# tayloraswift/swift-png

Hardware: AMD Instinct MI355X
Metric: decoded_mpixels_per_s (higher is better)
Workload: dtype u8

## Files before the change

### include/spng_mi355.h

```cpp
#ifndef SPNG_MI355_H
#define SPNG_MI355_H

#include <stddef.h>
#include <stdint.h>

#ifdef __cplusplus
extern "C" {
#endif

#define SPNG_VERSION 0x000100

enum {
    SPNG_DONE = 0,
    SPNG_NEED_MORE_INPUT = 1,
    SPNG_E_COMPRESSION_METHOD = 16,
    SPNG_E_WINDOW_SIZE = 17,
    SPNG_E_CHECK_BITS = 18,
    SPNG_E_DICTIONARY = 19,
    SPNG_E_STREAM_CHECKSUM = 32,
    SPNG_E_BLOCK_TYPE = 33,
    SPNG_E_BLOCK_COUNT_PARITY = 34,
    SPNG_E_RUNLITERAL_COUNT = 35,
    SPNG_E_CODELENGTH_TABLE = 36,
    SPNG_E_CODELENGTH_SEQUENCE = 37,
// ... 3 lines not shown
    SPNG_E_GZIP_METHOD = 25,
    SPNG_E_GZIP_FLAG_BITS = 26,
    SPNG_E_GZIP_HEADER_CHECKSUM = 27,
    SPNG_E_EXTRANEOUS_IMAGE_DATA = 48,
    SPNG_E_EXTRANEOUS_COMPRESSED_DATA = 49,
    SPNG_E_INCOMPLETE_DATASTREAM = 50,
    SPNG_E_TRUNCATED_SIGNATURE = 80,
    SPNG_E_SIGNATURE = 81,
    SPNG_E_TRUNCATED_CHUNK_HEADER = 82,
    SPNG_E_TRUNCATED_CHUNK_BODY = 83,
    SPNG_E_CHUNK_TYPE = 84,
    SPNG_E_CHUNK_CHECKSUM = 85,
    SPNG_E_TEXT_KEYWORD = 96,
    SPNG_E_TEXT_CHUNK_LENGTH = 97,
    SPNG_E_TEXT_LANGUAGE = 98,
    SPNG_E_TEXT_LOCALIZED_KEYWORD = 99,
    SPNG_E_TEXT_COMPRESSION_METHOD = 100,
    SPNG_E_TEXT_COMPRESSION = 101,
    SPNG_E_TEXT_INCOMPLETE = 102,
    SPNG_E_PROFILE_NAME = 104,
    SPNG_E_PROFILE_CHUNK_LENGTH = 105,
    SPNG_E_PROFILE_COMPRESSION_METHOD = 106,
    SPNG_E_PROFILE_INCOMPLETE = 107,
    SPNG_E_TEXT_ENCODING = 112,
    SPNG_E_OUTPUT_CAPACITY = 64,
    SPNG_E_ARGUMENT = 65,
    SPNG_E_DEVICE = 66,
    SPNG_E_REFERENCE_UNDEFINED = 67
};

enum { SPNG_FORMAT_ZLIB = 0,
       SPNG_FORMAT_IOS = 1,
       SPNG_FORMAT_GZIP = 2 };

typedef struct spng_ctx spng_ctx;

typedef struct spng_result {
    int32_t  status;
    int32_t  reserved;
    uint64_t written;
    uint64_t consumed;
    uint64_t aux[2];
} spng_result;

typedef struct spng_stream_desc {
    const void *d_src;  uint64_t src_len;
    void       *d_dst;  uint64_t dst_cap;
    int32_t     format;
    int32_t     reserved;
} spng_stream_desc;

typedef struct spng_image_desc {
    const void *d_idat;    uint64_t idat_len;
    void       *d_rows;    uint64_t rows_cap;
    void       *d_storage;
    uint32_t    width, height;
    uint8_t     depth;
    uint8_t     channels;
    uint8_t     interlaced;
    uint8_t     format;
    uint32_t    reserved;
} spng_image_desc;
enum { SPNG_IMAGE_OVERDRAW = 1 };

int32_t     spng_version(void);
const char *spng_status_string(int32_t status);
const char *spng_last_error_string(void);
uint64_t    spng_inflated_size(uint32_t w, uint32_t h, int depth, int channels, int interlaced);
uint64_t    spng_storage_size(uint32_t w, uint32_t h, int depth, int channels);

int32_t spng_create(int device, void *stream, spng_ctx **out);
void    spng_destroy(spng_ctx *ctx);
void   *spng_stream(spng_ctx *ctx);
int32_t spng_sync(spng_ctx *ctx);

enum { SPNG_CFG_INFLATE_MODE = 0,
       SPNG_CFG_SEGMENT_BYTES = 1,
       SPNG_CFG_TOKEN_BYTES = 2,
       SPNG_CFG_UNFILTER_PIECE_ROWS = 3,
       SPNG_CFG_RESOLVE_PARTS = 5,
       SPNG_CFG_DEFLATE_BYTES = 7,
       SPNG_CFG_MULTI_GROUPS = 8,
       SPNG_CFG_BLOCK_CUT_BYTES = 9,
       SPNG_CFG_COUNT = 10 };
enum { SPNG_BLOCK_CUT_AUTO = 0, SPNG_BLOCK_CUT_NEVER = 1 };
enum { SPNG_INFLATE_AUTO = 0, SPNG_INFLATE_SERIAL = 1 };
int32_t spng_configure(spng_ctx *ctx, int key, int64_t value);

enum { SPNG_K_INFLATE = 0,
       SPNG_K_UNFILTER = 1, SPNG_K_SCATTER = 2, SPNG_K_FILTER = 3,
       SPNG_K_DEFLATE = 4, SPNG_K_ADLER = 5,
       SPNG_K_PINFLATE = 6,
       SPNG_K_UNPACK = 7,
       SPNG_K_PACK = 10,
       SPNG_K_LEX = 12,
       SPNG_K_PINF_FIND = 8, SPNG_K_PINF_DECODE = 9, SPNG_K_PINF_RESOLVE = 11,
       SPNG_K_DFL_SEARCH = 13, SPNG_K_DFL_PARSE = 14,
       SPNG_K_ALPHA = 15,
       SPNG_K_CENSUS = 16,
       SPNG_K_PACK_INDEXED = 17,
       SPNG_K_HSVA = 18,
       SPNG_K_LUMINANCE = 19,
       SPNG_K_COUNT = 19 + 1 };
int32_t spng_profile(spng_ctx *ctx, int enable);
int32_t spng_profile_get(spng_ctx *ctx, int kernel, double *total_ms, uint64_t *launches);
int32_t spng_token_stats(spng_ctx *ctx, uint64_t *page_bytes, uint64_t *blocks, int32_t *ran_dry);
int32_t spng_cut_stats(spng_ctx *ctx, uint64_t *tried, uint64_t *joined, uint64_t *streams_redone);

int32_t spng_inflate_batch(spng_ctx *ctx, const spng_stream_desc *descs, uint32_t count,
                           spng_result *d_results, spng_result *h_results);

int32_t spng_inflate_resume_batch(spng_ctx *ctx, const spng_stream_desc *descs, const uint64_t *h_state, uint32_t count,
                                  spng_result *d_results, spng_result *h_results);

int32_t spng_unfilter_batch(spng_ctx *ctx, const spng_image_desc *descs, uint32_t count,
                            const uint64_t *d_rows_len,
                            spng_result *d_results, spng_result *h_results);

int32_t spng_decode_batch(spng_ctx *ctx, const spng_image_desc *descs, uint32_t count,
                          spng_result *d_results, spng_result *h_results);

int32_t spng_inflate(spng_ctx *ctx, const void *src, uint64_t n, int32_t format,
                     void *dst, uint64_t cap, spng_result *result);
int32_t spng_unfilter(spng_ctx *ctx, const void *rows, uint64_t rows_len,
                      uint32_t w, uint32_t h, int depth, int channels, int interlaced,
                      void *storage, spng_result *result);
int32_t spng_decode(spng_ctx *ctx, const void *idat, uint64_t n, int32_t format,
                    uint32_t w, uint32_t h, int depth, int channels, int interlaced,
                    void *storage, spng_result *result);
int32_t spng_adler32(spng_ctx *ctx, const void *data, uint64_t n, uint32_t *out);

typedef struct spng_file_desc {
    const void *d_png;  uint64_t len;
    void       *d_idat; uint64_t idat_cap;
} spng_file_desc;
typedef struct spng_lexed {
    int32_t  status;
    uint32_t chunks;
    uint64_t aux[2];
    uint32_t width, height;
    uint8_t  depth, color, compression, filter, interlace;
    uint8_t  ios;
    uint8_t  pad[2];
    uint64_t idat_len;
    uint64_t plte_off, trns_off;
    uint32_t plte_len, trns_len;
    uint64_t consumed;
} spng_lexed;
int32_t spng_lex_batch(spng_ctx *ctx, const spng_file_desc *files, uint32_t count,
                       spng_lexed *d_infos, spng_lexed *h_infos);
uint64_t spng_lex_state_bytes(void);
int32_t spng_lex_resume_batch(spng_ctx *ctx, const spng_file_desc *files, void *const *d_states, uint32_t count,
                              spng_lexed *d_infos, spng_lexed *h_infos);
int32_t spng_lex_resume_stats(spng_ctx *ctx, uint64_t *summed, uint64_t *copied, uint64_t *headers);
#define SPNG_NO_OFFSET 0xffffffffu
typedef struct spng_chunk_entry {
    uint32_t type;
    uint32_t length;
    uint64_t offset;
    int32_t  status;
    uint32_t aux;
    uint32_t k, l, m;
    uint32_t body_off;
    uint8_t  compressed;
    uint8_t  pad[7];
} spng_chunk_entry;
typedef struct spng_chunk_dir {
    spng_chunk_entry *d_entries;
    uint32_t          cap;
    uint32_t          reserved;
} spng_chunk_dir;
int32_t spng_lex_dir_batch(spng_ctx *ctx, const spng_file_desc *files, const spng_chunk_dir *dirs, uint32_t count,
                           spng_lexed *d_infos, spng_lexed *h_infos);

enum { SPNG_TEXT_LATIN1_TO_UTF8 = 1,
       SPNG_TEXT_CHECK_UTF8 = 2 };
typedef struct spng_text_desc {
    const void *d_in;   uint64_t len;
    void       *d_out;  uint64_t out_cap;
    uint8_t     op;
    uint8_t     reserved[7];
} spng_text_desc;
int32_t spng_text_batch(spng_ctx *ctx, const spng_text_desc *descs, uint32_t count, spng_result *d_results, spng_result *h_results);

typedef struct spng_chunking_desc {
    const void *d_stream; uint64_t len;
    void       *d_out;    uint64_t out_cap;
    uint64_t    chunk_bytes;
} spng_chunking_desc;
int32_t spng_write_idat_batch(spng_ctx *ctx, const spng_chunking_desc *descs, uint32_t count,
// ... 205 lines not shown
```

### swift_png_amd/__init__.py

```python
from __future__ import annotations

import ctypes
import os
from pathlib import Path

_HERE = Path(__file__).resolve().parent
LIB_PATH = Path(os.environ.get("SPNG_LIB", _HERE / "libspng_mi355.so"))

DONE, NEED_MORE_INPUT = 0, 1
E_COMPRESSION_METHOD, E_WINDOW_SIZE, E_CHECK_BITS, E_DICTIONARY = 16, 17, 18, 19
E_GZIP_SIGIL, E_GZIP_METHOD, E_GZIP_FLAG_BITS, E_GZIP_HEADER_CHECKSUM = 24, 25, 26, 27
(E_STREAM_CHECKSUM, E_BLOCK_TYPE, E_BLOCK_COUNT_PARITY, E_RUNLITERAL_COUNT, E_CODELENGTH_TABLE,
 E_CODELENGTH_SEQUENCE, E_HUFFMAN_TABLE, E_STRING_REFERENCE) = range(32, 40)
E_EXTRANEOUS_IMAGE_DATA, E_EXTRANEOUS_COMPRESSED_DATA, E_INCOMPLETE_DATASTREAM = 48, 49, 50
E_OUTPUT_CAPACITY, E_ARGUMENT, E_DEVICE, E_REFERENCE_UNDEFINED = 64, 65, 66, 67
(E_TRUNCATED_SIGNATURE, E_SIGNATURE, E_TRUNCATED_CHUNK_HEADER, E_TRUNCATED_CHUNK_BODY, E_CHUNK_TYPE,
 E_CHUNK_CHECKSUM) = range(80, 86)
(E_TEXT_KEYWORD, E_TEXT_CHUNK_LENGTH, E_TEXT_LANGUAGE, E_TEXT_LOCALIZED_KEYWORD, E_TEXT_COMPRESSION_METHOD, E_TEXT_COMPRESSION,
 E_TEXT_INCOMPLETE) = range(96, 103)
E_PROFILE_NAME, E_PROFILE_CHUNK_LENGTH, E_PROFILE_COMPRESSION_METHOD, E_PROFILE_INCOMPLETE = range(104, 108)
E_TEXT_ENCODING = 112
NO_OFFSET = 0xffffffff
TEXT_LATIN1_TO_UTF8, TEXT_CHECK_UTF8 = 1, 2
TEXT_TILE = 4096
FORMAT_ZLIB, FORMAT_IOS, FORMAT_GZIP = 0, 1, 2
K_INFLATE, K_UNFILTER, K_SCATTER, K_FILTER, K_DEFLATE, K_ADLER, K_PINFLATE = 0, 1, 2, 3, 4, 5, 6
K_UNPACK = 7
K_PACK = 10
IMAGE_OVERDRAW = 1
TARGET_RGBA, TARGET_VA, TARGET_SCALAR = 0, 1, 2
PREMULTIPLY, PREMULTIPLY_AS_U8, STRAIGHTEN, STRAIGHTEN_AS_U8 = 1, 2, 3, 4
K_LEX = 12
K_PINF_FIND, K_PINF_DECODE, K_PINF_RESOLVE = 8, 9, 11
K_DFL_SEARCH, K_DFL_PARSE = 13, 14
K_ALPHA = 15
K_CENSUS, K_PACK_INDEXED = 16, 17
K_HSVA = 18
HSVA_FROM_RGBA8, HSVA_TO_RGBA8, HSVA_TO_VA8 = 1, 2, 3
_HSVA_BYTES = {1: (4, 8), 2: (8, 4), 3: (8, 2)}
K_LUMINANCE = 19
LUMINANCE_V8, LUMINANCE_VA8 = 1, 2
CENSUS_LDS_SLOTS, CENSUS_LDS_LIMIT = 2048, 512
CENSUS_FINISH_LDS_KEYS = 4096
PACK_INDEXED_LDS_KEYS = 512
CENSUS_WIDE_CAP = 1 << 24
CENSUS_WIDE_TILE = 4096
MAP_LDS_KEYS, MAP_LDS_SLOTS = 512, 2048
MAP_MIN_SLOTS = 64
CFG_INFLATE_MODE, CFG_SEGMENT_BYTES, CFG_TOKEN_BYTES, CFG_UNFILTER_PIECE_ROWS, CFG_RESOLVE_PARTS = 0, 1, 2, 3, 5
CFG_DEFLATE_BYTES, CFG_MULTI_GROUPS = 7, 8
CFG_BLOCK_CUT_BYTES = 9
BLOCK_CUT_AUTO, BLOCK_CUT_NEVER = 0, 1
INFLATE_AUTO, INFLATE_SERIAL = 0, 1

EXPORTS = [
    "spng_version", "spng_status_string", "spng_last_error_string", "spng_inflated_size",
    "spng_storage_size", "spng_create", "spng_destroy", "spng_stream", "spng_sync", "spng_profile",
    "spng_profile_get", "spng_token_stats", "spng_cut_stats", "spng_configure", "spng_inflate_batch", "spng_inflate_resume_batch", "spng_unfilter_batch",
    "spng_unfilter_resume_batch", "spng_decode_batch",
    "spng_inflate", "spng_unfilter", "spng_decode", "spng_adler32", "spng_filter_batch", "spng_filter",
    "spng_lex_batch", "spng_write_idat_batch", "spng_crc32", "spng_unpack_batch", "spng_unpack", "spng_unpack_as", "spng_pack_batch", "spng_pack_as", "spng_alpha_batch", "spng_alpha", "spng_hsva_batch", "spng_hsva", "spng_luminance_batch", "spng_luminance", "spng_census_batch", "spng_census", "spng_pack_indexed_batch", "spng_pack_indexed", "spng_census_wide_batch", "spng_census_wide", "spng_map_batch", "spng_map", "spng_deflate_bound", "spng_deflate_batch", "spng_deflate", "spng_deflate_window", "spng_encode_batch",
    "spng_shard", "spng_decode_batch_multi", "spng_copy_ceiling", "spng_trim", "spng_lds_exchange_ordered", "spng_deflate_state_bytes", "spng_deflate_resume_batch",
    "spng_lex_state_bytes", "spng_lex_resume_batch", "spng_lex_resume_stats",
    "spng_file_bound", "spng_write_file_batch", "spng_compress_batch",
    "spng_lex_dir_batch", "spng_text_batch",
]


def source_digest() -> str:
    import hashlib
    h = hashlib.sha256()
    root = Path(__file__).resolve().parent
    for f in sorted(list((root / "csrc").glob("*.hip")) + list((root / "csrc").glob("*.hpp")) + list((root.parent / "include").glob("*.h"))):
        h.update(f.name.encode()); h.update(f.read_bytes())
    return h.hexdigest()[:16]


class Result(ctypes.Structure):
    _fields_ = [("status", ctypes.c_int32), ("reserved", ctypes.c_int32), ("written", ctypes.c_uint64),
                ("consumed", ctypes.c_uint64), ("aux", ctypes.c_uint64 * 2)]


class StreamDesc(ctypes.Structure):
    _fields_ = [("d_src", ctypes.c_void_p), ("src_len", ctypes.c_uint64), ("d_dst", ctypes.c_void_p),
                ("dst_cap", ctypes.c_uint64), ("format", ctypes.c_int32), ("reserved", ctypes.c_int32)]


class ImageDesc(ctypes.Structure):
    _fields_ = [("d_idat", ctypes.c_void_p), ("idat_len", ctypes.c_uint64), ("d_rows", ctypes.c_void_p),
                ("rows_cap", ctypes.c_uint64), ("d_storage", ctypes.c_void_p), ("width", ctypes.c_uint32),
                ("height", ctypes.c_uint32), ("depth", ctypes.c_uint8), ("channels", ctypes.c_uint8),
                ("interlaced", ctypes.c_uint8), ("format", ctypes.c_uint8), ("reserved", ctypes.c_uint32)]


class FileDesc(ctypes.Structure):
    _fields_ = [("d_png", ctypes.c_void_p), ("len", ctypes.c_uint64), ("d_idat", ctypes.c_void_p), ("idat_cap", ctypes.c_uint64)]


class Lexed(ctypes.Structure):
    _fields_ = [("status", ctypes.c_int32), ("chunks", ctypes.c_uint32), ("aux", ctypes.c_uint64 * 2),
                ("width", ctypes.c_uint32), ("height", ctypes.c_uint32), ("depth", ctypes.c_uint8), ("color", ctypes.c_uint8),
                ("compression", ctypes.c_uint8), ("filter", ctypes.c_uint8), ("interlace", ctypes.c_uint8),
                ("ios", ctypes.c_uint8), ("pad", ctypes.c_uint8 * 2), ("idat_len", ctypes.c_uint64),
                ("plte_off", ctypes.c_uint64), ("trns_off", ctypes.c_uint64), ("plte_len", ctypes.c_uint32),
                ("trns_len", ctypes.c_uint32), ("consumed", ctypes.c_uint64)]


class ChunkEntry(ctypes.Structure):
    _fields_ = [("type", ctypes.c_uint32), ("length", ctypes.c_uint32), ("offset", ctypes.c_uint64), ("status", ctypes.c_int32),
                ("aux", ctypes.c_uint32), ("k", ctypes.c_uint32), ("l", ctypes.c_uint32), ("m", ctypes.c_uint32),
                ("body_off", ctypes.c_uint32), ("compressed", ctypes.c_uint8), ("pad", ctypes.c_uint8 * 7)]


class ChunkDir(ctypes.Structure):
    _fields_ = [("d_entries", ctypes.c_void_p), ("cap", ctypes.c_uint32), ("reserved", ctypes.c_uint32)]


class TextDesc(ctypes.Structure):
    _fields_ = [("d_in", ctypes.c_void_p), ("len", ctypes.c_uint64), ("d_out", ctypes.c_void_p), ("out_cap", ctypes.c_uint64),
                ("op", ctypes.c_uint8), ("reserved", ctypes.c_uint8 * 7)]


class UnpackDesc(ctypes.Structure):
    _fields_ = [("d_storage", ctypes.c_void_p), ("d_out", ctypes.c_void_p), ("d_palette", ctypes.c_void_p),
                ("width", ctypes.c_uint32), ("height", ctypes.c_uint32), ("palette_count", ctypes.c_uint32),
                ("key", ctypes.c_uint16 * 3), ("depth", ctypes.c_uint8), ("channels", ctypes.c_uint8), ("indexed", ctypes.c_uint8),
                ("bgr", ctypes.c_uint8), ("has_key", ctypes.c_uint8), ("target", ctypes.c_uint8), ("layout", ctypes.c_uint8),
                ("premultiply", ctypes.c_uint8), ("reserved", ctypes.c_uint8 * 6)]


class PackDesc(ctypes.Structure):
    _fields_ = [("d_pixels", ctypes.c_void_p), ("d_storage", ctypes.c_void_p), ("d_palette", ctypes.c_void_p),
                ("width", ctypes.c_uint32), ("height", ctypes.c_uint32), ("palette_count", ctypes.c_uint32),
                ("depth", ctypes.c_uint8), ("channels", ctypes.c_uint8), ("indexed", ctypes.c_uint8), ("bgr", ctypes.c_uint8),
                ("source", ctypes.c_uint8), ("layout", ctypes.c_uint8), ("premultiply", ctypes.c_uint8),
                ("reserved", ctypes.c_uint8 * 5)]


class AlphaDesc(ctypes.Structure):
    _fields_ = [("d_in", ctypes.c_void_p), ("d_out", ctypes.c_void_p), ("count", ctypes.c_uint64), ("bits", ctypes.c_uint8),
                ("layout", ctypes.c_uint8), ("op", ctypes.c_uint8), ("reserved", ctypes.c_uint8 * 5)]
# ... 101 lines not shown


class DecodingError(SpngError):
    pass


class LexingError(SpngError):
    pass


class ParsingError(SpngError):
    pass


_NAMES = {
    16: "invalidCompressionMethod", 17: "invalidWindowSize", 18: "invalidCheckBits", 19: "unexpectedDictionary",
    24: "invalidSigil", 25: "invalidCompressionMethod", 26: "invalidFlagBits", 27: "_headerChecksumUnsupported",
    32: "invalidStreamChecksum", 33: "invalidBlockTypeCode", 34: "invalidBlockElementCountParity",
    35: "invalidHuffmanRunLiteralSymbolCount", 36: "invalidHuffmanCodelengthHuffmanTable",
    37: "invalidHuffmanCodelengthSequence", 38: "invalidHuffmanTable", 39: "invalidStringReference",
    48: "extraneousImageData", 49: "extraneousImageDataCompressedData",
    50: "incompleteImageDataCompressedDatastream", 64: "outputCapacity", 65: "invalidArgument",
    66: "deviceError", 67: "referenceUndefined",
    80: "truncatedSignature", 81: "invalidSignature", 82: "truncatedChunkHeader", 83: "truncatedChunkBody",
    84: "invalidChunkTypeCode", 85: "invalidChunkChecksum",
    96: "invalidTextEnglishKeyword", 97: "invalidTextChunkLength", 98: "invalidTextLanguageTag", 99: "invalidTextLocalizedKeyword",
    100: "invalidTextCompressionMethodCode", 101: "invalidTextCompressionCode", 102: "incompleteTextCompressedDatastream",
    104: "invalidColorProfileName", 105: "invalidColorProfileChunkLength", 106: "invalidColorProfileCompressionMethodCode",
    107: "incompleteColorProfileCompressedDatastream", 112: "textEncoding",
}


def raise_for(status, aux=(0, 0)):
    if status in (DONE, NEED_MORE_INPUT):
        return
    if 24 <= status < 28:
        raise GzipStreamHeaderError(status, aux)
    if 16 <= status < 32:
        raise StreamHeaderError(status, aux)
    if 32 <= status < 48:
        raise DecompressionError(status, aux)
    if 48 <= status < 64:
        raise DecodingError(status, aux)
    if 80 <= status < 96:
        raise LexingError(status, aux)
    if 96 <= status < 112:
        raise ParsingError(status, aux)
    raise SpngError(status, aux)


_lib = None


def load_library():
    global _lib
    if _lib is not None:
        return _lib
    if not LIB_PATH.exists():
        raise RuntimeError(f"{LIB_PATH} is missing: run `python -c 'import __graft_entry__ as g; g.build()'` "
                           "(hipcc --offload-arch=gfx950); there is no CPU fallback")
    import torch
    lib = ctypes.CDLL(str(LIB_PATH))
    vp, u64, u32, i32 = ctypes.c_void_p, ctypes.c_uint64, ctypes.c_uint32, ctypes.c_int32
    rp = ctypes.POINTER(Result)
    lib.spng_version.restype = i32
    lib.spng_status_string.restype = ctypes.c_char_p
    lib.spng_status_string.argtypes = [i32]
    lib.spng_last_error_string.restype = ctypes.c_char_p
    lib.spng_inflated_size.restype = u64
    lib.spng_inflated_size.argtypes = [u32, u32, ctypes.c_int, ctypes.c_int, ctypes.c_int]
    lib.spng_storage_size.restype = u64
    lib.spng_storage_size.argtypes = [u32, u32, ctypes.c_int, ctypes.c_int]
    lib.spng_create.argtypes = [ctypes.c_int, vp, ctypes.POINTER(vp)]
    lib.spng_destroy.restype = None
    lib.spng_destroy.argtypes = [vp]
    lib.spng_stream.restype = vp
    lib.spng_stream.argtypes = [vp]
    lib.spng_sync.argtypes = [vp]
    lib.spng_configure.argtypes = [vp, ctypes.c_int, ctypes.c_int64]
    lib.spng_profile.argtypes = [vp, ctypes.c_int]
    lib.spng_profile_get.argtypes = [vp, ctypes.c_int, ctypes.POINTER(ctypes.c_double), ctypes.POINTER(u64)]
    lib.spng_token_stats.argtypes = [vp, ctypes.POINTER(u64), ctypes.POINTER(u64), ctypes.POINTER(ctypes.c_int32)]
    lib.spng_cut_stats.argtypes = [vp, ctypes.POINTER(u64), ctypes.POINTER(u64), ctypes.POINTER(u64)]
    lib.spng_inflate_batch.argtypes = [vp, ctypes.POINTER(StreamDesc), u32, vp, rp]
    lib.spng_inflate_resume_batch.argtypes = [vp, ctypes.POINTER(StreamDesc), ctypes.POINTER(ctypes.c_uint64), u32, vp, rp]
    lib.spng_unfilter_batch.argtypes = [vp, ctypes.POINTER(ImageDesc), u32, vp, vp, rp]
    lib.spng_unfilter_resume_batch.argtypes = [vp, ctypes.POINTER(ImageDesc), ctypes.POINTER(ctypes.c_void_p), ctypes.POINTER(u64),
                                               ctypes.POINTER(u64), u32, vp, rp]
    lib.spng_decode_batch.argtypes = [vp, ctypes.POINTER(ImageDesc), u32, vp, rp]
    lib.spng_filter_batch.argtypes = [vp, ctypes.POINTER(ImageDesc), u32, vp, rp]
    lib.spng_inflate.argtypes = [vp, vp, u64, i32, vp, u64, rp]
    lib.spng_unfilter.argtypes = [vp, vp, u64, u32, u32, ctypes.c_int, ctypes.c_int, ctypes.c_int, vp, rp]
    lib.spng_decode.argtypes = [vp, vp, u64, i32, u32, u32, ctypes.c_int, ctypes.c_int, ctypes.c_int, vp, rp]
    lib.spng_adler32.argtypes = [vp, vp, u64, ctypes.POINTER(u32)]
    lib.spng_filter.argtypes = [vp, vp, u32, u32, ctypes.c_int, ctypes.c_int, ctypes.c_int, vp, rp]
    lib.spng_lex_batch.argtypes = [vp, ctypes.POINTER(FileDesc), u32, vp, ctypes.POINTER(Lexed)]
    lib.spng_lex_state_bytes.restype = u64
    lib.spng_lex_resume_batch.argtypes = [vp, ctypes.POINTER(FileDesc), ctypes.POINTER(vp), u32, vp, ctypes.POINTER(Lexed)]
    lib.spng_lex_dir_batch.argtypes = [vp, ctypes.POINTER(FileDesc), ctypes.POINTER(ChunkDir), u32, vp, ctypes.POINTER(Lexed)]
    lib.spng_text_batch.argtypes = [vp, ctypes.POINTER(TextDesc), u32, vp, rp]
    lib.spng_lex_resume_stats.argtypes = [vp, ctypes.POINTER(u64), ctypes.POINTER(u64), ctypes.POINTER(u64)]
    lib.spng_write_idat_batch.argtypes = [vp, ctypes.POINTER(ChunkingDesc), u32, vp, rp]
    lib.spng_crc32.argtypes = [vp, vp, u64, ctypes.POINTER(u32)]
    lib.spng_file_bound.restype = u64
    lib.spng_file_bound.argtypes = [ctypes.POINTER(PngDesc), u64]
    lib.spng_write_file_batch.argtypes = [vp, ctypes.POINTER(PngDesc), u32, vp, rp]
    lib.spng_compress_batch.argtypes = [vp, ctypes.POINTER(ImageDesc), ctypes.POINTER(PngDesc), i32, u32, vp, rp]
    lib.spng_unpack_batch.argtypes = [vp, vp, u32]
    lib.spng_unpack.argtypes = [vp, vp, u32, u32, ctypes.c_int, ctypes.c_int, ctypes.c_int, ctypes.c_int, ctypes.c_int,
                                vp, u32, vp, vp]
    lib.spng_unpack_as.argtypes = [vp, vp, u32, u32, ctypes.c_int, ctypes.c_int, ctypes.c_int, ctypes.c_int, ctypes.c_int,
                                   ctypes.c_int, ctypes.c_int, vp, u32, vp, vp]
    lib.spng_pack_batch.argtypes = [vp, vp, u32]
    lib.spng_pack_as.argtypes = [vp, vp, u32, u32, ctypes.c_int, ctypes.c_int, ctypes.c_int, ctypes.c_int, ctypes.c_int,
                                 ctypes.c_int, vp, u32, vp]
    lib.spng_alpha_batch.argtypes = [vp, vp, u32, vp, rp]
    lib.spng_alpha.argtypes = [vp, vp, u64, ctypes.c_int, ctypes.c_int, ctypes.c_int, vp, rp]
    lib.spng_hsva_batch.argtypes = [vp, vp, u32, vp, rp]
    lib.spng_hsva.argtypes = [vp, vp, u64, ctypes.c_int, vp, rp]
    lib.spng_luminance_batch.argtypes = [vp, vp, u32, vp, rp]
    lib.spng_luminance.argtypes = [vp, vp, u64, ctypes.c_int, vp, rp]
    lib.spng_census_batch.argtypes = [vp, vp, u32, vp, rp]
    lib.spng_census.argtypes = [vp, vp, u64, ctypes.c_int, ctypes.c_int, ctypes.c_int, u32, vp, vp, rp]
    lib.spng_pack_indexed_batch.argtypes = [vp, vp, u32, vp, rp]
    lib.spng_pack_indexed.argtypes = [vp, vp, u32, u32, ctypes.c_int, ctypes.c_int, ctypes.c_int, vp, vp, u32, ctypes.c_int, vp, rp]
    lib.spng_census_wide_batch.argtypes = [vp, vp, u32, vp, rp]
    lib.spng_census_wide.argtypes = [vp, vp, u64, ctypes.c_int, ctypes.c_int, ctypes.c_int, u32, vp, vp, rp]
    lib.spng_map_batch.argtypes = [vp, vp, u32, vp, rp]
    lib.spng_map.argtypes = [vp, vp, u64, ctypes.c_int, ctypes.c_int, ctypes.c_int, vp, vp, u32, ctypes.c_int, vp, vp, rp]
    lib.spng_deflate_bound.restype = u64
    lib.spng_deflate_bound.argtypes = [u64]
    lib.spng_deflate_batch.argtypes = [vp, ctypes.POINTER(StreamDesc), ctypes.POINTER(i32), u32, vp, rp]
    lib.spng_deflate.argtypes = [vp, vp, u64, i32, i32, vp, u64, rp]
    lib.spng_deflate_window.argtypes = [vp, vp, u64, i32, i32, i32, vp, u64, rp]
    lib.spng_encode_batch.argtypes = [vp, ctypes.POINTER(ImageDesc), i32, u32, vp, rp]
    lib.spng_deflate_state_bytes.restype = u64
    lib.spng_deflate_resume_batch.argtypes = [vp, ctypes.POINTER(StreamDesc), ctypes.POINTER(i32), ctypes.POINTER(vp), ctypes.POINTER(ctypes.c_uint8),
                                              ctypes.POINTER(u64), u32, vp, rp]
    lib.spng_shard.argtypes = [u32, u32, u32, ctypes.POINTER(u32), ctypes.POINTER(u32)]
    lib.spng_decode_batch_multi.argtypes = [ctypes.POINTER(vp), u32, ctypes.POINTER(ImageDesc), u32, ctypes.POINTER(vp), rp]
    lib.spng_copy_ceiling.argtypes = [vp, vp, vp, u64, i32, i32, ctypes.POINTER(ctypes.c_double)]
    lib.spng_trim.argtypes = [vp]
    for name in EXPORTS:
        getattr(lib, name)
    _lib = lib
    return lib


_sessions = {}


def load(device: int = 0) -> "Session":
    if device not in _sessions:
        _sessions[device] = Session(device)
    return _sessions[device]


def shard_of(count: int, parts: int, index: int):
    first, n = ctypes.c_uint32(0), ctypes.c_uint32(0)
    lib = load_library()
    _check(lib, lib.spng_shard(count, parts, index, ctypes.byref(first), ctypes.byref(n)))
    return first.value, n.value


def decode_batch_multi(sessions, descs, gather=None):
    lib = load_library()
# ... 71 lines not shown
        i = int(index(key_aggregate(int(k), layout)))
        if not 0 <= i <= 255:
            raise OverflowError(f"indexer returned {i} for {key_aggregate(int(k), layout)}: not representable in UInt8")
        out[j] = i
    return bytes(out)


def tabulate_deindexer(dereference, layout=TARGET_RGBA) -> bytes:
    out = bytearray(1024)
    for i in range(256):
        v = dereference(i)
        if layout == TARGET_RGBA:
            q = tuple(v)
        elif layout == TARGET_VA:
            q = (v[0], v[0], v[0], v[1])
        else:
            q = (v, v, v, 255)
        if len(q) != 4 or not all(0 <= int(x) <= 255 for x in q):
            raise OverflowError(f"deindexer returned {v!r} for {i}: UInt8 components are needed")
        out[4 * i:4 * i + 4] = bytes(int(x) for x in q)
    return bytes(out)


class Session:

    def __init__(self, device: int = 0, use_torch_stream: bool = True):
        import torch
        if not torch.cuda.is_available():
            raise RuntimeError("swift_png_amd needs an MI355X (gfx950); no HIP device is visible and there is "
                               "no CPU fallback")
        self.torch = torch
        self.lib = load_library()
        self.device = device
        self.tdev = torch.device("cuda", device)
        handle = ctypes.c_void_p()
        stream = None
        if use_torch_stream:
            with torch.cuda.device(device):
                stream = ctypes.c_void_p(torch.cuda.current_stream().cuda_stream)
        _check(self.lib, self.lib.spng_create(device, stream, ctypes.byref(handle)))
        self.ctx = handle

    def close(self):
        if self.ctx:
            self.lib.spng_destroy(self.ctx)
            self.ctx = None

    def sync(self):
        _check(self.lib, self.lib.spng_sync(self.ctx))

    def configure(self, key, value):
        _check(self.lib, self.lib.spng_configure(self.ctx, key, int(value)))

    def profile(self, enable=True):
        _check(self.lib, self.lib.spng_profile(self.ctx, int(enable)))

    def trim(self):
        _check(self.lib, self.lib.spng_trim(self.ctx))

    def copy_ceiling(self, nbytes=8 << 30, pattern=0, repeats=5):
        t = self.torch
        a = t.zeros(nbytes // 8, dtype=t.int64, device=self.tdev)
        b = t.empty(nbytes // 8, dtype=t.int64, device=self.tdev)
        ms = ctypes.c_double(0)
        _check(self.lib, self.lib.spng_copy_ceiling(self.ctx, b.data_ptr(), a.data_ptr(), nbytes, pattern, repeats, ctypes.byref(ms)))
        del a, b
        return 2 * nbytes / (ms.value * 1e-3) / 1e9, ms.value

    def profile_get(self, kernel):
        ms, n = ctypes.c_double(0), ctypes.c_uint64(0)
        _check(self.lib, self.lib.spng_profile_get(self.ctx, kernel, ctypes.byref(ms), ctypes.byref(n)))
        return ms.value, n.value

    def token_stats(self):
        b, k, d = ctypes.c_uint64(0), ctypes.c_uint64(0), ctypes.c_int32(0)
        _check(self.lib, self.lib.spng_token_stats(self.ctx, ctypes.byref(b), ctypes.byref(k), ctypes.byref(d)))
        return b.value, k.value, bool(d.value)

    def cut_stats(self):
        t, j, r = ctypes.c_uint64(0), ctypes.c_uint64(0), ctypes.c_uint64(0)
        _check(self.lib, self.lib.spng_cut_stats(self.ctx, ctypes.byref(t), ctypes.byref(j), ctypes.byref(r)))
        return t.value, j.value, r.value

    def to_device(self, data):
        t = self.torch
        if isinstance(data, (bytes, bytearray, memoryview)):
            if len(data) == 0:
                return t.empty(0, dtype=t.uint8, device=self.tdev)
            return t.frombuffer(bytearray(data), dtype=t.uint8).to(self.tdev)
        return t.as_tensor(data, dtype=t.uint8).to(self.tdev)

    def empty(self, n):
        return self.torch.empty(max(int(n), 1), dtype=self.torch.uint8, device=self.tdev)

    @staticmethod
    def _ptr(tensor):
        return ctypes.c_void_p(tensor.data_ptr() if tensor is not None and tensor.numel() else None)

    def inflate_batch(self, streams, caps, fmt=FORMAT_ZLIB):
        n = len(streams)
        outs = [self.empty(c) for c in caps]
        descs = (StreamDesc * n)()
        for i, (s, o, c) in enumerate(zip(streams, outs, caps)):
            descs[i] = StreamDesc(self._ptr(s), s.numel(), self._ptr(o), int(c), pick(fmt, i), 0)
        res = (Result * n)()
        _check(self.lib, self.lib.spng_inflate_batch(self.ctx, descs, n, None, res))
        return outs, list(res)

    def inflate_resume(self, src, src_len, dst, fmt=FORMAT_ZLIB, state=(0, 0, 0, 0)):
        desc = (StreamDesc * 1)(StreamDesc(self._ptr(src), int(src_len), self._ptr(dst), dst.numel(), fmt, 0))
        state = tuple(state) + (0, 0) * (len(state) == 2)
        st = (ctypes.c_uint64 * 4)(*[int(v) for v in state])
        res = (Result * 1)()
        _check(self.lib, self.lib.spng_inflate_resume_batch(self.ctx, desc, st, 1, None, res))
        r = res[0]
        if r.status == NEED_MORE_INPUT:
            tok = int(r.consumed)
            return r, (int(r.aux[0]), int(r.aux[1]), tok, int(r.written) if tok else 0)
        return r, tuple(state)

    def unfilter_resume(self, desc, work, prev_len, now_len):
        arr = (ImageDesc * 1)(desc)
        wp = (ctypes.c_void_p * 1)(self._ptr(work) if work is not None else None)
        prev, now = (ctypes.c_uint64 * 1)(int(prev_len)), (ctypes.c_uint64 * 1)(int(now_len))
        res = (Result * 1)()
        _check(self.lib, self.lib.spng_unfilter_resume_batch(self.ctx, arr, wp, prev, now, 1, None, res))
        return res[0]

    def image_desc(self, idat, rows, storage, w, h, depth, channels, interlaced, fmt=FORMAT_ZLIB, rows_cap=None):
        return ImageDesc(self._ptr(idat), idat.numel() if idat is not None else 0, self._ptr(rows),
                         int(rows_cap if rows_cap is not None else rows.numel()), self._ptr(storage),
                         w, h, depth, channels, int(bool(interlaced)), fmt, 0)

    def decode_batch(self, descs, wait=True):
        n = len(descs)
        arr = descs if isinstance(descs, ctypes.Array) else (ImageDesc * n)(*descs)
        if wait:
            res = (Result * n)()
            _check(self.lib, self.lib.spng_decode_batch(self.ctx, arr, n, None, res))
            return list(res)
        if getattr(self, "_dres", None) is None or self._dres.numel() < n * ctypes.sizeof(Result):
            self._dres = self.empty(n * ctypes.sizeof(Result))
        _check(self.lib, self.lib.spng_decode_batch(self.ctx, arr, n, self._ptr(self._dres), None))
        return None

    def fetch_results(self, n):
        raw = bytes(self._dres[:n * ctypes.sizeof(Result)].cpu().numpy())
        return list((Result * n).from_buffer_copy(raw))

    def unfilter_batch(self, descs, rows_len=None):
        n = len(descs)
        arr = (ImageDesc * n)(*descs)
        res = (Result * n)()
        dl = None
        if rows_len is not None:
            dl = self.torch.tensor(list(rows_len), dtype=self.torch.int64, device=self.tdev)
        _check(self.lib, self.lib.spng_unfilter_batch(self.ctx, arr, n, self._ptr(dl) if dl is not None else None,
                                                      None, res))
        return list(res)

    def filter_batch(self, descs):
        n = len(descs)
        arr = (ImageDesc * n)(*descs)
        res = (Result * n)()
        _check(self.lib, self.lib.spng_filter_batch(self.ctx, arr, n, None, res))
        return list(res)
# ... 483 lines not shown
```

### swift_png_amd/csrc/api.hip

```cpp
#include "host.hpp"

namespace spng {

thread_local char g_err[512] = "";

int passes(uint32_t w, uint32_t h, int volume, int interlaced, Pass out[7])
{
    static const uint32_t A7[7][4] = {{0, 0, 3, 3}, {4, 0, 3, 3}, {0, 4, 2, 3}, {2, 0, 2, 2},
                                      {0, 2, 1, 2}, {1, 0, 1, 1}, {0, 1, 0, 1}};
    int n = 0;
    if (!interlaced) {
        if (w && h) out[n++] = Pass{0, 0, 1, 1, w, h, ((uint64_t)w * volume + 7) >> 3};
        return n;
    }
    for (int z = 0; z < 7; ++z) {
        const uint32_t bx = A7[z][0], by = A7[z][1], ex = A7[z][2], ey = A7[z][3];
        const uint32_t sx = 1u << ex, sy = 1u << ey;
        if (w + sx - bx - 1 < sx || h + sy - by - 1 < sy) continue;
        const uint32_t sw = (w + sx - bx - 1) >> ex, sh = (h + sy - by - 1) >> ey;
        if (!sw || !sh) continue;
        out[n++] = Pass{bx, by, sx, sy, sw, sh, ((uint64_t)sw * volume + 7) >> 3};
    }
    return n;
}
// ... 53 lines not shown
    default: return "unknown status";
    }
}

const char *spng_last_error_string(void) { return g_err; }

uint64_t spng_inflated_size(uint32_t w, uint32_t h, int depth, int channels, int interlaced)
{
    Pass p[7];
    const int n = passes(w, h, depth * channels, interlaced, p);
    uint64_t u = 0;
    for (int i = 0; i < n; ++i) u += (p[i].pitch + 1) * (uint64_t)p[i].h;
    return u;
}

uint64_t spng_storage_size(uint32_t w, uint32_t h, int depth, int channels)
{
    return (uint64_t)w * h * (uint64_t)((depth * channels + 7) >> 3);
}

int32_t spng_create(int device, void *stream, spng_ctx **out)
{
    if (!out) return SPNG_E_ARGUMENT;
    *out = nullptr;
    int count = 0;
    hipError_t e = hipGetDeviceCount(&count);
    if (e != hipSuccess || device < 0 || device >= count)
        return fail_hip(e == hipSuccess ? hipErrorInvalidDevice : e, "spng_create: no such HIP device");
    hipDeviceProp_t prop;
    HIP_TRY(hipGetDeviceProperties(&prop, device));
    if (strncmp(prop.gcnArchName, "gfx950", 6) != 0) {
        snprintf(g_err, sizeof g_err, "spng_create: device %d is %s; this library contains gfx950 code only",
                 device, prop.gcnArchName);
        return SPNG_E_DEVICE;
    }
    HIP_TRY(hipSetDevice(device));
    spng_ctx *c = new spng_ctx;
    c->device = device;
    if (stream) c->stream = (hipStream_t)stream;
    else {
        hipError_t e2 = hipStreamCreateWithFlags(&c->stream, hipStreamNonBlocking);
        if (e2 != hipSuccess) { delete c; return fail_hip(e2, "hipStreamCreateWithFlags"); }
        c->owns_stream = true;
    }
    if (hipError_t e3 = launch_deflate3_probe(c->stream); e3 != hipSuccess) { (void)hipGetLastError(); }
    *out = c;
    return SPNG_DONE;
}

void spng_destroy(spng_ctx *c)
{
    if (!c) return;
    (void)hipSetDevice(c->device);
    (void)hipStreamSynchronize(c->stream);
    for (auto &s : c->spans) { (void)hipEventDestroy(s.a); (void)hipEventDestroy(s.b); }
    for (auto e : c->pool) (void)hipEventDestroy(e);
    if (c->d_ws) (void)hipFree(c->d_ws);
    for (auto &sl : c->slabs) { if (sl.h) (void)hipHostFree(sl.h); if (sl.ev) (void)hipEventDestroy(sl.ev); }
    for (auto b : c->batch_buffers()) if (*b.p) (void)hipFree(*b.p);
    if (c->h_pool_used) (void)hipHostFree(c->h_pool_used);
    if (c->h_lex_stats) (void)hipHostFree(c->h_lex_stats);
    if (c->pool_ev) (void)hipEventDestroy(c->pool_ev);
    if (c->stream2) { (void)hipStreamSynchronize(c->stream2); (void)hipStreamDestroy(c->stream2); }
    if (c->stream_out) { (void)hipStreamSynchronize(c->stream_out); (void)hipStreamDestroy(c->stream_out); }
    for (hipEvent_t e : c->ev_out) if (e) (void)hipEventDestroy(e);
    for (hipEvent_t e : {c->ev_fork, c->ev_join}) if (e) (void)hipEventDestroy(e);
    for (hipEvent_t e : c->ev_dfl) if (e) (void)hipEventDestroy(e);
    if (c->owns_stream) (void)hipStreamDestroy(c->stream);
    delete c;
}

void *spng_stream(spng_ctx *c) { return c ? (void *)c->stream : nullptr; }

int32_t spng_sync(spng_ctx *c)
{
    if (!c) return SPNG_E_ARGUMENT;
    HIP_TRY(hipStreamSynchronize(c->stream));
    return SPNG_DONE;
}

int32_t spng_configure(spng_ctx *c, int key, int64_t value)
{
    if (!c || key < 0 || key >= SPNG_CFG_COUNT || key == 4 || key == 6  || value < 0) return SPNG_E_ARGUMENT;
    std::lock_guard<std::mutex> g(c->mu);
    c->cfg[key] = value;
    return SPNG_DONE;
}

int32_t spng_profile(spng_ctx *c, int enable)
{
    if (!c) return SPNG_E_ARGUMENT;
    std::lock_guard<std::mutex> g(c->mu);
    HIP_TRY(hipStreamSynchronize(c->stream));
    for (auto &s : c->spans) { c->pool.push_back(s.a); c->pool.push_back(s.b); }
    c->spans.clear();
    c->profiling = enable != 0;
    return SPNG_DONE;
}

int32_t spng_token_stats(spng_ctx *c, uint64_t *page_bytes, uint64_t *blocks, int32_t *ran_dry)
{
    if (!c) return SPNG_E_ARGUMENT;
    std::lock_guard<std::mutex> g(c->mu);
    HIP_TRY(hipSetDevice(c->device));
    HIP_TRY(hipStreamSynchronize(c->stream));
    const uint32_t *h = c->h_pool_used;
    if (page_bytes) *page_bytes = h ? (uint64_t)h[0] << 16 : 0;
    if (ran_dry) *ran_dry = h ? (int32_t)h[1] : 0;
    if (blocks) *blocks = h ? h[2] : 0;
    return SPNG_DONE;
}

int32_t spng_cut_stats(spng_ctx *c, uint64_t *tried, uint64_t *joined, uint64_t *streams_redone)
{
    if (!c) return SPNG_E_ARGUMENT;
    std::lock_guard<std::mutex> g(c->mu);
    HIP_TRY(hipSetDevice(c->device));
    HIP_TRY(hipStreamSynchronize(c->stream));
    const uint32_t *h = c->h_pool_used && c->cut_stats_valid ? c->h_pool_used + 8 : nullptr;
    if (tried) *tried = h ? h[0] : 0;
    if (joined) *joined = h ? h[1] : 0;
    if (streams_redone) *streams_redone = h ? h[2] : 0;
    return SPNG_DONE;
}

int32_t spng_profile_get(spng_ctx *c, int kernel, double *total_ms, uint64_t *launches)
{
    if (!c || kernel < 0 || kernel >= SPNG_K_COUNT) return SPNG_E_ARGUMENT;
    std::lock_guard<std::mutex> g(c->mu);
    HIP_TRY(hipStreamSynchronize(c->stream));
    double t = 0; uint64_t n = 0;
    for (auto &s : c->spans) if (s.kernel == kernel) {
        float ms = 0;
        HIP_TRY(hipEventElapsedTime(&ms, s.a, s.b));
        t += ms; ++n;
    }
    if (total_ms) *total_ms = t;
    if (launches) *launches = n;
    return SPNG_DONE;
}

}

extern "C" {

int32_t spng_copy_ceiling(spng_ctx *c, void *d_dst, const void *d_src, uint64_t bytes, int32_t pattern, int32_t repeats, double *ms_per_copy)
{
    if (!c || !d_dst || !d_src || bytes < 65536 || pattern < 0 || pattern > 1 || repeats < 1 || !ms_per_copy) return SPNG_E_ARGUMENT;
    HIP_TRY(hipSetDevice(c->device));
    std::lock_guard<std::mutex> g(c->mu);
    hipEvent_t e0 = c->event(), e1 = c->event();
    HIP_TRY(launch_copy_probe(d_src, d_dst, bytes, pattern, c->stream));
    HIP_TRY(hipEventRecord(e0, c->stream));
    for (int32_t i = 0; i < repeats; ++i) HIP_TRY(launch_copy_probe(d_src, d_dst, bytes, pattern, c->stream));
    HIP_TRY(hipEventRecord(e1, c->stream));
    HIP_TRY(hipEventSynchronize(e1));
    float ms = 0;
    HIP_TRY(hipEventElapsedTime(&ms, e0, e1));
    c->pool.push_back(e0); c->pool.push_back(e1);
    *ms_per_copy = (double)ms / repeats;
    return SPNG_DONE;
}

int32_t spng_lds_exchange_ordered(spng_ctx *c, int32_t *ordered)
{
    if (!c || !ordered) return SPNG_E_ARGUMENT;
    HIP_TRY(hipSetDevice(c->device));
    std::lock_guard<std::mutex> g(c->mu);
    HIP_TRY(hipStreamSynchronize(c->stream));
    uint32_t v = 0;
    HIP_TRY(deflate3_probe_result(&v));
    *ordered = (int32_t)v;
    return SPNG_DONE;
}

int32_t spng_trim(spng_ctx *c)
{
    if (!c) return SPNG_E_ARGUMENT;
    HIP_TRY(hipSetDevice(c->device));
    std::lock_guard<std::mutex> g(c->mu);
    HIP_TRY(hipStreamSynchronize(c->stream));
    if (c->stream2) HIP_TRY(hipStreamSynchronize(c->stream2));
    if (c->stream_out) HIP_TRY(hipStreamSynchronize(c->stream_out));
    for (auto b : c->batch_buffers()) {
        if (*b.p) HIP_TRY(hipFree(*b.p));
        *b.p = nullptr; *b.cap = 0;
    }
    c->pool_ratio = 0; c->block_bytes = 0; c->sym_failed = 0;
    return SPNG_DONE;
}

int32_t spng_shard(uint32_t count, uint32_t parts, uint32_t index, uint32_t *first, uint32_t *n)
{
    if (!parts || index >= parts || !first || !n) return SPNG_E_ARGUMENT;
    const uint32_t per = (count + parts - 1) / parts;
    const uint64_t lo = (uint64_t)per * index;
    *first = lo < count ? (uint32_t)lo : count;
    *n = lo >= count ? 0u : (count - lo < per ? count - (uint32_t)lo : per);
    return SPNG_DONE;
}

}
```

### swift_png_amd/csrc/common.hpp

```cpp
#pragma once
#include <hip/hip_runtime.h>
#include <stdint.h>
#include "../../include/spng_mi355.h"

namespace spng {

#define UNI(x) ((uint32_t)__builtin_amdgcn_readfirstlane((int)(x)))
__device__ __forceinline__ uint64_t uni64(uint64_t v) { return (uint64_t)UNI(v >> 32) << 32 | UNI((uint32_t)v); }
#define UB(c) (UNI((c) ? 1u : 0u) != 0u)
#ifndef SPNG_EMU
typedef uint8_t __attribute__((address_space(1))) gbyte;
#else
typedef uint8_t gbyte;
#endif

struct SpinGuard {
    uint32_t spins = 0;
    uint64_t t0 = 0;
    __device__ __forceinline__ void tick()
    {
        if ((++spins & 0xfffu) != 0) return;
#ifndef SPNG_EMU
        const uint64_t now = __builtin_amdgcn_s_memrealtime();
        if (!t0) t0 = now;
// ... 114 lines not shown
    unsigned long long *sort;
    spng_result   *result;
    uint32_t       cap, slots, slot_bits;
    uint8_t        layout, premultiply, pad[2];
};

struct PackIndexedJob {
    const void    *pixels;
    uint8_t       *storage;
    const uint32_t *keys;
    const uint8_t *indices;
    spng_result   *result;
    uint32_t       width, height;
    uint32_t       map_count;
    uint8_t        layout, premultiply, miss, pad;
};

struct MapJob {
    const void    *pixels;
    void          *out;
    const uint32_t *keys;
    const void    *values;
    spng_result   *result;
    uint64_t       count;
    uint64_t       miss;
    uint64_t       table_off;
    uint32_t       map_count, slots, slot_bits;
    uint8_t        layout, premultiply, value_bytes, pad;
};

struct FileJob {
    const uint8_t *head;
    const uint8_t *stream;
    const spng_result *src_result;
    uint8_t       *out;
    uint32_t      *partial;
    uint64_t       head_len, len, stream_cap, out_cap, chunk_bytes;
};

struct TextJob {
    const uint8_t *in;
    uint8_t       *out;
    uint64_t       len, out_cap;
    uint64_t       tiles;
    uint32_t      *counts;
    uint32_t      *firsts;
    uint64_t      *offs;
    uint8_t        op, pad[7];
};

struct InflateJob {
    const uint8_t *src;
    uint8_t       *dst;
    uint64_t       src_len;
    uint64_t       dst_cap;
    int32_t        format;
    uint32_t       image;
    const int32_t *skip;
    uint64_t      *state;
    uint32_t       internal, pad;
};

struct PStream {
    const uint8_t *src;
    uint8_t       *dst;
    uint64_t       src_len, dst_cap;
    int32_t        format;
    uint32_t       image;
    uint32_t       seg_first, seg_count;
    uint64_t       seg_bytes;
    uint64_t       tok_base, ntok;
    uint64_t       end_bit;
    int32_t        ok;
    uint32_t       pass;
    uint64_t       start_bit, out_pos;
    uint64_t      *state;
    uint32_t       serial_only, cut_segs;
    uint32_t       parts_max, parts;
    uint64_t       out_total;
    uint64_t       sym_off;
    uint32_t       cut_on, cut_resumed;
    uint64_t       seg_origin, tok_bit, blk_out;
    uint64_t       ho_hdr, ho_out;
};
enum { PSEG_FAIL = 0, PSEG_CONT = 1, PSEG_FINAL = 2, PSEG_PARTIAL = 3, PSEG_NOPAGE = 4,
       PSEG_CUT = 5 };
static constexpr uint64_t RESUME_SERIAL_BITS = 8ull << 20;
static constexpr uint32_t PCUT_RECS = 4;
struct PSeg {
    uint32_t stream, index;
    uint64_t log_off, log_cap;
    uint64_t start_bit;
    uint64_t end_bit;
    uint64_t ntok;
    uint64_t tok_base;
    int32_t  status;
    uint32_t used;
    uint32_t next, head;
    uint64_t nbytes;
    uint64_t out_base;
};
struct PCut {
    uint32_t cut, anchor;
    uint32_t nrec, joined;
    uint32_t next_head, tbl_here;
    uint64_t tbl, tbl_id;
    uint64_t head_tbl;
    uint64_t add_tok, add_bytes;
    uint64_t next_sub;
    uint64_t tbl_bytes;
    uint64_t next_bit;
    uint64_t join_tbl, join_tbl_bytes;
    struct { uint64_t bit; uint32_t hw, bytes; } rec[PCUT_RECS];
};
struct PPart {
    uint32_t seg, seg_end;
    uint64_t out_pos;
    uint64_t out_len;
    unsigned long long sumS, sumI;
    uint32_t present, failed;
};

struct DeflateJob {
    const uint8_t *src;
    uint8_t       *dst;
    uint64_t       src_len;
    uint64_t       dst_cap;
    int32_t        format, level;
    uint32_t       image;
    uint32_t       exponent;
    uint32_t       more;
    struct D1State *state;
    uint64_t       plan_pos;
    uint32_t       plan_limit, pad2;
    uint64_t       plan_aux;
};

struct D1State {
    uint64_t w, inserted;
    uint64_t acc, total;
    uint32_t nacc, overflow, count, started;
    uint32_t adlerS, adlerI, pad[2];
    uint32_t terms[2048];
    uint64_t rb, re, srb, sre, spos;
    uint32_t done, pad3;
};
struct D3Stream {
    const uint8_t *src; uint8_t *dst;
    uint64_t src_len, dst_cap;
    int32_t  format, level;
    uint32_t image, exponent;
    uint32_t more, pad;
    D1State *state;
    uint32_t *match[2];
    uint32_t *terms;
    uint32_t *bdesc;
    uint64_t *bbits;
    uint8_t  *scratch;
};

struct D2State {
    uint64_t rb, re;
    uint64_t pos;
    uint32_t limit, generic;
    uint64_t acc, total;
    uint32_t nacc, overflow;
    uint32_t adlerS, adlerI;
    uint32_t fail, done;
    uint8_t  depths[544];
    uint32_t started, pad;
    uint64_t srb, sre, spos;
    uint32_t slimit, spad;
};
struct D2Stream {
    const uint8_t *src; uint8_t *dst;
    uint64_t src_len, dst_cap;
    int32_t  format, level;
    uint32_t image, exponent;
    uint32_t more, pad;
    D2State *state;
    uint16_t *vinfo; uint64_t *bbase; uint32_t *bwords; uint64_t *emask;
    uint16_t *vinfo2; uint64_t *bbase2; uint32_t *bwords2;
    uint32_t *up, *step; uint8_t *pathb, *litb;
};

struct Pass { uint32_t bx, by, sx, sy, w, h; uint64_t pitch; };
int passes(uint32_t w, uint32_t h, int volume, int interlaced, Pass out[7]);

template <class Launch> inline hipError_t launch_rows(uint32_t count, Launch launch)
{
    for (uint32_t y0 = 0; y0 < count; y0 += 65535u) launch(y0, count - y0 < 65535u ? count - y0 : 65535u);
    return hipGetLastError();
}

hipError_t launch_unfilter(const UnfJob *d_jobs, uint32_t count, uint32_t bpp, spng_result *d_results,
                           uint32_t pieces, uint32_t piece_rows, hipStream_t stream, uint32_t widest = 0);
hipError_t launch_copy_probe(const void *d_src, void *d_dst, uint64_t bytes, int pattern, hipStream_t stream);
hipError_t launch_scatter(const ScatterJob *d_jobs, uint32_t count, const uint32_t *d_job_image,
                          const spng_result *d_results, uint32_t blocks_x, hipStream_t stream);
hipError_t launch_overdraw(const OverdrawJob *d_jobs, uint32_t count, uint32_t blocks_x, hipStream_t stream);
hipError_t launch_inflate(const InflateJob *d_jobs, uint32_t count, spng_result *d_results,
                          hipStream_t stream);
hipError_t launch_pinf2_find(PStream *d_streams, PSeg *d_segs, uint32_t seg0, uint32_t nsegs, uint32_t retry, hipStream_t stream);
hipError_t launch_pinf2_decode(PStream *d_streams, PSeg *d_segs, uint32_t seg0, uint32_t nsegs, uint32_t *d_pt, uint8_t *d_pool, uint32_t *d_next,
                               uint32_t pages, uint32_t retry, hipStream_t stream);
hipError_t launch_pinf2_scan(PStream *d_streams, uint32_t nstreams, PSeg *d_segs, PPart *d_parts, uint32_t retry, hipStream_t stream);
hipError_t launch_pinf2_resolve(PStream *d_streams, uint32_t nstreams, PSeg *d_segs, uint32_t *d_pt, uint8_t *d_pool, uint32_t pages,
                                spng_result *d_results, int32_t *d_done, PPart *d_parts, uint32_t pmax, uint32_t retry, hipStream_t stream);
hipError_t launch_pinf2_parts(PStream *d_streams, uint32_t nstreams, PSeg *d_segs, uint32_t *d_pt, uint8_t *d_pool, uint32_t pages,
                              spng_result *d_results, int32_t *d_done, PPart *d_parts, uint32_t pmax, uint16_t *d_sym, hipStream_t stream);
hipError_t launch_pinf2_join(PStream *d_streams, uint32_t nstreams, spng_result *d_results, int32_t *d_done, PPart *d_parts, uint32_t pmax,
                             uint16_t *d_sym, uint8_t *d_win, hipStream_t stream);
hipError_t launch_pinf2_cutplan(PStream *d_streams, uint32_t nstreams, PSeg *d_segs, PCut *d_cuts, uint32_t *d_stats, hipStream_t stream);
hipError_t launch_pinf2_cutdecode(PStream *d_streams, PSeg *d_segs, PCut *d_cuts, uint32_t seg0, uint32_t nsegs, uint32_t *d_pt, uint8_t *d_pool,
                                  uint32_t *d_next, uint32_t pages, hipStream_t stream);
hipError_t launch_pinf2_cutjoin(PStream *d_streams, PSeg *d_segs, PCut *d_cuts, uint32_t seg0, uint32_t nsegs, uint32_t *d_pt, uint8_t *d_pool,
                                uint32_t *d_next, uint32_t pages, uint32_t *d_stats, hipStream_t stream);
hipError_t launch_pinf2_cutscan(PStream *d_streams, uint32_t nstreams, PSeg *d_segs, PCut *d_cuts, PPart *d_parts, uint32_t *d_stats, hipStream_t stream);
hipError_t launch_pinf2_account(uint32_t *d_ctr, uint32_t *d_totals, uint32_t pages, hipStream_t stream);
static constexpr uint64_t GZ_NONE = ~0ull;
uint32_t   gzip_pieces();
hipError_t launch_gzip_pre(InflateJob *d_jobs, PStream *d_streams, spng_result *d_results, uint64_t *d_gz, int32_t *d_done,
                           uint32_t count, hipStream_t stream);
hipError_t launch_gzip_inflate_post(const InflateJob *d_jobs, spng_result *d_results, const uint64_t *d_gz, uint32_t *d_parts,
                                    uint32_t count, hipStream_t stream);
hipError_t launch_gzip_deflate_post(const DeflateJob *d_jobs, spng_result *d_results, uint32_t *d_parts, uint32_t count,
                                    hipStream_t stream);
hipError_t launch_resume_post(const InflateJob *d_jobs, spng_result *d_results, uint64_t *d_parts, uint32_t count, hipStream_t stream);
uint64_t deflate_state_bytes();
uint32_t deflate2_plan(uint64_t n, bool more, uint64_t &pos, uint32_t &lim);
hipError_t launch_deflate2_begin(const D2Stream *d_streams, uint32_t count, hipStream_t stream);
uint64_t deflate2_vertices(uint64_t n);
hipError_t launch_deflate2_search(const D2Stream *d_streams, uint32_t count, uint32_t cps, uint32_t chunk_len, uint32_t *d_pool, unsigned long long *d_pool_next,
                                  uint64_t pool_words, uint32_t *d_temp, uint32_t parity, hipStream_t stream);
uint64_t deflate2_temp_bytes(uint32_t workgroups);
uint64_t deflate3_round_positions();
uint64_t deflate3_end(uint64_t n, bool more);
hipError_t launch_deflate3_begin(const D3Stream *d_streams, uint32_t count, hipStream_t stream);
hipError_t launch_deflate3_search(const D3Stream *d_streams, uint32_t count, uint32_t cps, uint32_t chunk_len, uint32_t parity, hipStream_t stream);
hipError_t launch_deflate3_probe(hipStream_t stream);
hipError_t deflate3_probe_result(uint32_t *ordered);
hipError_t launch_deflate3_parse(const D3Stream *d_streams, uint32_t count, spng_result *d_results, uint32_t parity, hipStream_t stream);
uint64_t deflate4_max_blocks(uint64_t positions);
uint64_t deflate4_block_bytes();
hipError_t launch_deflate4_round(const D3Stream *d_streams, uint32_t count, uint32_t max_blocks, spng_result *d_results, uint32_t parity, hipStream_t stream);
hipError_t launch_deflate2_parse(const D2Stream *d_streams, uint32_t count, const uint32_t *d_pool, spng_result *d_results, uint32_t parity, hipStream_t stream);
hipError_t launch_deflate2_failed(const D2Stream *d_streams, uint32_t count, uint32_t *d_failed, hipStream_t stream);
hipError_t launch_unpack(const UnpackJob *d_jobs, uint32_t count, uint32_t blocks_x, int target, hipStream_t stream);
hipError_t launch_pack(const PackJob *d_jobs, uint32_t count, uint32_t blocks_x, int source, hipStream_t stream);
hipError_t launch_alpha(const AlphaJob *d_jobs, uint32_t count, uint32_t blocks_x, int bits, hipStream_t stream);
hipError_t launch_hsva(const HsvaJob *d_jobs, uint32_t count, uint32_t blocks_x, hipStream_t stream);
hipError_t launch_luminance(const LuminanceJob *d_jobs, uint32_t count, uint32_t blocks_x, hipStream_t stream);
uint32_t census_slots(uint32_t cap);
uint32_t census_sort_elems(uint32_t cap);
hipError_t launch_census(const CensusJob *d_jobs, uint32_t count, uint32_t blocks_x, int bits, hipStream_t stream);
hipError_t launch_pack_indexed(const PackIndexedJob *d_jobs, uint32_t count, uint32_t blocks_x, int source, hipStream_t stream);
hipError_t launch_census_count(const CensusJob *d_jobs, uint32_t count, uint32_t blocks_x, int bits, hipStream_t stream);
hipError_t launch_census_wide_finish(const CensusJob *d_jobs, uint32_t count, uint32_t most_slots, uint32_t most_keys, hipStream_t stream);
uint32_t map_slots(uint32_t map_count);
hipError_t launch_map(const MapJob *d_jobs, uint32_t count, unsigned long long *d_scratch, uint32_t build_blocks_x, uint32_t blocks_x,
                      int source, hipStream_t stream);
size_t lex_chunk_bytes();
size_t lex_walk_bytes();
hipError_t launch_lex(const spng_file_desc *d_files, uint32_t count, spng_lexed *d_out, void *d_table, const uint64_t *d_table_at,
                      void *d_walks, uint32_t max_listed, hipStream_t stream);
hipError_t launch_lex_dir(const spng_file_desc *d_files, const spng_chunk_dir *d_dirs, uint32_t count, const spng_lexed *d_out, const void *d_table,
                          const uint64_t *d_table_at, const void *d_walks, uint32_t most_entries, hipStream_t stream);
size_t text_tiles(uint64_t len);
hipError_t launch_text(const TextJob *d_jobs, uint32_t count, uint32_t blocks_x, bool writes, spng_result *d_results, hipStream_t stream);
size_t lex_state_bytes();
size_t lex_piece_bytes();
size_t lex_rwalk_bytes();
hipError_t launch_lex_resume(const spng_file_desc *d_files, void *const *d_states, uint32_t count, spng_lexed *d_out, void *d_table,
                             const uint64_t *d_table_at, void *d_walks, uint32_t max_listed, uint64_t *d_stats, hipStream_t stream);
hipError_t launch_write_idat(const spng_chunking_desc *d_descs, uint32_t count, uint32_t blocks_x, spng_result *d_results, hipStream_t stream);
hipError_t launch_write_file(const FileJob *d_jobs, uint32_t count, uint32_t blocks_x, uint64_t finish_chunks, spng_result *d_results,
                             hipStream_t stream);
hipError_t launch_crc_partial(const uint8_t *d, uint64_t n, uint64_t piece, uint32_t *d_partial, uint32_t pieces, hipStream_t stream);
uint32_t crc32_fold(const uint32_t *partial, uint64_t pieces, uint64_t n, uint64_t piece);
hipError_t launch_filter(const FilterJob *d_jobs, uint32_t count, uint32_t max_rows, hipStream_t stream);
hipError_t launch_adler_partial(const uint8_t *d, uint64_t n, uint32_t chunk, uint64_t *d_out, uint32_t blocks,
                                hipStream_t stream);

}
```

### swift_png_amd/csrc/host.hpp

```cpp
#pragma once
#include "common.hpp"
#include <stdio.h>
#include <stdlib.h>
#include <string.h>
#include <algorithm>
#include <array>
#include <functional>
#include <mutex>
#include <vector>

namespace spng {

extern thread_local char g_err[512];

static int32_t fail_hip(hipError_t e, const char *what)
{
    snprintf(g_err, sizeof g_err, "%s: %s", what, hipGetErrorString(e));
    return SPNG_E_DEVICE;
}
static int32_t fail_text(const char *what)
{
    snprintf(g_err, sizeof g_err, "%s", what);
    return SPNG_E_DEVICE;
}
#define HIP_TRY(expr) do { hipError_t e_ = (expr); if (e_ != hipSuccess) return fail_hip(e_, #expr); } while (0)

static bool valid_format(int depth, int channels)
{
    if (channels < 1 || channels > 4) return false;
    if (depth == 8 || depth == 16) return true;
    return channels == 1 && (depth == 1 || depth == 2 || depth == 4);
}

__global__ void init_results_kernel(spng_result *results, const uint64_t *written, uint32_t count);

}

using namespace spng;

struct spng_ctx {
    int device = 0;
    hipStream_t stream = nullptr;
    bool owns_stream = false;
    void *d_ws = nullptr;  size_t d_ws_cap = 0;
    static constexpr int SLABS = 4;
    struct Slab { void *h = nullptr; size_t cap = 0; hipEvent_t ev = nullptr; bool pending = false; };
    Slab slabs[SLABS];
    int slab_next = 0;
    void *h_ws = nullptr;
    Slab *cur = nullptr;
    void *d_graph = nullptr; size_t graph_cap = 0;
    void *d_log = nullptr;  size_t log_cap = 0;
    void *d_tok = nullptr;  size_t tok_cap = 0;
    void *d_sym = nullptr;  size_t sym_cap = 0;
    uint64_t sym_failed = 0;
    void *d_win = nullptr;  size_t win_cap = 0;
    void *d_census = nullptr; size_t census_cap = 0;
    void *d_file = nullptr;  size_t file_cap = 0;
    double   pool_ratio = 0;
    uint32_t *h_pool_used = nullptr;
    bool cut_stats_valid = false;
    uint64_t pool_pages_planned = 0, pool_src_bytes = 0, pool_src_pending = 0;
    double   block_bytes = 0;
    hipEvent_t pool_ev = nullptr; bool pool_pending = false;
    uint64_t *h_lex_stats = nullptr;
    hipEvent_t ev_dfl[4] = {nullptr, nullptr, nullptr, nullptr};
    hipStream_t stream2 = nullptr;
    hipEvent_t ev_fork = nullptr, ev_join = nullptr;
    hipStream_t stream_out = nullptr;
    hipEvent_t ev_out[2] = {nullptr, nullptr};
    void *d_multi = nullptr; size_t multi_cap = 0;
    uint64_t peers = 0, peers_refused = 0;
    int64_t cfg[SPNG_CFG_COUNT] = {0, 0, 0, 0, 0, 0, 0, 0, 0};
    bool profiling = false;
    struct Span { int kernel; hipEvent_t a, b; };
    std::vector<Span> spans;
    std::vector<hipEvent_t> pool;
    std::mutex mu;

    struct Buf { void **p; size_t *cap; };
    std::array<Buf, 8> batch_buffers()
    {
        return {{{&d_graph, &graph_cap}, {&d_log, &log_cap}, {&d_tok, &tok_cap}, {&d_sym, &sym_cap}, {&d_win, &win_cap}, {&d_multi, &multi_cap},
                 {&d_census, &census_cap}, {&d_file, &file_cap}}};
    }
    int32_t grow(void *&buf, size_t &cap, size_t need, size_t slack, bool *failed = nullptr)
    {
        if (failed) *failed = false;
        if (need <= cap) return SPNG_DONE;
        HIP_TRY(hipStreamSynchronize(stream));
        if (buf) { HIP_TRY(hipFree(buf)); buf = nullptr; }
        cap = 0;
        const hipError_t e = hipMalloc(&buf, need + slack);
        if (e != hipSuccess) {
            buf = nullptr;
            if (!failed) return fail_hip(e, "hipMalloc");
            (void)hipGetLastError();
            *failed = true;
            return SPNG_DONE;
        }
        cap = need + slack;
        return SPNG_DONE;
    }
    int32_t reserve(size_t bytes)
    {
        if (int32_t st = grow(d_ws, d_ws_cap, bytes, bytes / 2 + 4096)) return st;
        Slab &sl = slabs[slab_next];
        slab_next = (slab_next + 1) % SLABS;
        if (sl.pending) { HIP_TRY(hipEventSynchronize(sl.ev)); sl.pending = false; }
        if (bytes > sl.cap) {
            if (sl.h) { HIP_TRY(hipHostFree(sl.h)); sl.h = nullptr; sl.cap = 0; }
            const size_t cap = bytes + bytes / 2 + 4096;
            HIP_TRY(hipHostMalloc(&sl.h, cap, hipHostMallocDefault));
            sl.cap = cap;
        }
        if (!sl.ev) HIP_TRY(hipEventCreateWithFlags(&sl.ev, hipEventDisableTiming));
        cur = &sl; h_ws = sl.h;
        return SPNG_DONE;
    }
    int32_t upload(size_t from, size_t to)
    {
        if (to > from)
            HIP_TRY(hipMemcpyAsync((char *)d_ws + from, (char *)h_ws + from, to - from, hipMemcpyHostToDevice, stream));
        HIP_TRY(hipEventRecord(cur->ev, stream));
        cur->pending = true;
        return SPNG_DONE;
    }
    hipEvent_t event()
    {
        if (!pool.empty()) { hipEvent_t e = pool.back(); pool.pop_back(); return e; }
        hipEvent_t e = nullptr;
        (void)hipEventCreate(&e);
        return e;
    }
};

static int32_t second_stream(spng_ctx *c)
{
    if (c->stream2) return SPNG_DONE;
    HIP_TRY(hipStreamCreateWithFlags(&c->stream2, hipStreamNonBlocking));
    for (hipEvent_t *e : {&c->ev_fork, &c->ev_join}) HIP_TRY(hipEventCreateWithFlags(e, hipEventDisableTiming));
    return SPNG_DONE;
}

static int32_t read_back(spng_ctx *c, void *h, const void *d, size_t bytes)
{
    if (!h) return SPNG_DONE;
    HIP_TRY(hipMemcpyAsync(h, d, bytes, hipMemcpyDeviceToHost, c->stream));
    HIP_TRY(hipStreamSynchronize(c->stream));
    return SPNG_DONE;
}

struct Timed {
    spng_ctx *c; int k; hipEvent_t a = nullptr; hipStream_t s;
    Timed(spng_ctx *c_, int k_, hipStream_t s_ = nullptr) : c(c_), k(k_), s(s_ ? s_ : c_->stream) { if (c->profiling) { a = c->event(); (void)hipEventRecord(a, s); } }
    ~Timed() { if (a) { hipEvent_t b = c->event(); (void)hipEventRecord(b, s); c->spans.push_back({k, a, b}); } }
// ... 18 lines not shown
```

### swift_png_amd/csrc/host_decode.hip

```cpp
#include "host.hpp"
#include "geometry.hpp"

namespace spng {

__global__ void finish_decode_kernel(spng_result *results, const uint64_t *expected, uint32_t count)
{
    const uint32_t i = blockIdx.x * blockDim.x + threadIdx.x;
    if (i >= count) return;
    const int32_t st = results[i].status;
    if (st == SPNG_E_OUTPUT_CAPACITY ||
        ((st == SPNG_DONE || st == SPNG_NEED_MORE_INPUT) && results[i].written > expected[i]))
        results[i].status = SPNG_E_EXTRANEOUS_IMAGE_DATA;
}

__global__ void poison_results_kernel(spng_result *results, uint32_t count)
{
    const uint32_t i = blockIdx.x * blockDim.x + threadIdx.x;
    if (i >= count) return;
    results[i].status = SPNG_E_DEVICE; results[i].reserved = 0;
    results[i].written = 0; results[i].consumed = 0;
    results[i].aux[0] = results[i].aux[1] = 0;
}

__global__ void init_results_kernel(spng_result *results, const uint64_t *written, uint32_t count)
// ... 95 lines not shown
                const UnfilterPieces cut = unfilter_pieces((uint32_t)k, total_rows, max_rows, widest, (uint32_t)c->cfg[SPNG_CFG_UNFILTER_PIECE_ROWS]);
                HIP_TRY(launch_unfilter(a.dev<UnfJob>(slots.unf[k]), (uint32_t)plan.unf[k].size(), k,
                                        d_results, cut.pieces, cut.piece_rows, c->stream, (uint32_t)(widest > 0xffffffffull ? 0xffffffffull : widest)));
            }
    }
    if (!plan.scat.empty()) {
        Timed t(c, SPNG_K_SCATTER);
        uint64_t maxpix = 1;
        for (auto &s : plan.scat) { uint64_t px = (uint64_t)s.sub_w * s.sub_h; if (px > maxpix) maxpix = px; }
        HIP_TRY(launch_scatter(a.dev<ScatterJob>(slots.scat), (uint32_t)plan.scat.size(),
                               a.dev<uint32_t>(slots.scat_image), d_results, plane_blocks_x(maxpix, SCATTER_BLOCKS_MAX), c->stream));
    }
    if (!plan.over.empty()) {
        Timed t(c, SPNG_K_SCATTER);
        uint64_t maxpix = 1;
        for (auto &o : plan.over) { uint64_t px = (uint64_t)o.width * (o.y1 - o.y0); if (px > maxpix) maxpix = px; }
        HIP_TRY(launch_overdraw(a.dev<OverdrawJob>(slots.over), (uint32_t)plan.over.size(), plane_blocks_x(maxpix, OVERDRAW_BLOCKS_MAX), c->stream));
    }
    return SPNG_DONE;
}

struct InflatePlan {
    std::vector<InflateJob> jobs;
    std::vector<PStream> streams;
    std::vector<PSeg> segs;
    size_t log_bytes = 0;
    bool parallel = false;
    uint32_t pool_pages = 0;
    struct Group { uint32_t s0, s1, g0, g1; };
    std::vector<Group> groups;
    std::vector<uint64_t> est;
    uint32_t pmax = 0;
    size_t parts_at = 0;
    size_t next_at = 0;
    bool gzip = false;
    std::vector<uint64_t> state;
    bool internal = true;
    size_t jobs_at = 0, streams_at = 0, segs_at = 0, done_at = 0, gz_at = 0, gzparts_at = 0, state_at = 0, sumparts_at = 0;
    bool cuts = false;
    size_t cuts_at = 0;
    size_t take_cuts(Arena &a) { if (cuts) cuts_at = a.take(segs.size() * sizeof(PCut)); return cuts_at; }
    size_t bytes() const
    {
        return jobs.size() * (sizeof(InflateJob) + sizeof(PStream) + 4 + (size_t)pmax * sizeof(PPart) + 256 + (gzip ? 8 + 4 * (size_t)gzip_pieces() : 0) +
                              (state.empty() ? 0 : 32 + 8 * (size_t)gzip_pieces())) +
               segs.size() * (sizeof(PSeg) + (cuts ? sizeof(PCut) : 0)) + 8192 + 1024;
    }
};

#ifndef SPNG_PARTS_MAX
#define SPNG_PARTS_MAX 128
#endif

static int32_t learn_from_last_batch(spng_ctx *c, uint64_t total)
{
    if (c->pool_pending && c->pool_ratio == 0 && hipEventQuery(c->pool_ev) != hipSuccess) {
        size_t free_b = 0, total_b = 0;
        HIP_TRY(hipMemGetInfo(&free_b, &total_b));
        uint64_t room = c->cfg[SPNG_CFG_TOKEN_BYTES] ? (uint64_t)c->cfg[SPNG_CFG_TOKEN_BYTES] : (uint64_t)(free_b + c->tok_cap) / 2;
        if ((double)total * 3.2 > (double)room) HIP_TRY(hipEventSynchronize(c->pool_ev));
    }
    if (c->pool_pending && hipEventQuery(c->pool_ev) == hipSuccess) {
        c->pool_pending = false;
        const uint64_t used = c->h_pool_used[0], blocks = c->h_pool_used[2];
        if (c->h_pool_used[1]) c->pool_ratio = 0;
        else if (c->pool_src_pending > (1u << 20)) c->pool_ratio = (double)used * 65536.0 / (double)c->pool_src_pending;
        c->block_bytes = (blocks && c->pool_src_pending > (1u << 20)) ? (double)c->pool_src_pending / (double)blocks : 0;
    }
    return SPNG_DONE;
}

static int32_t cut_into_segments(spng_ctx *c, InflatePlan &p, uint64_t seg_bytes)
{
    p.streams.resize(p.jobs.size());
    const double per_byte = c->pool_ratio > 0 ? (c->pool_ratio * 1.25 < 1.0 ? 1.0 : c->pool_ratio * 1.25) : 3.2;
    p.est.assign(p.jobs.size(), 0);
    size_t log = 0;
    for (size_t i = 0; i < p.jobs.size(); ++i) {
        const InflateJob &j = p.jobs[i];
        PStream &st = p.streams[i];
        memset(&st, 0, sizeof st);
        st.src = j.src; st.dst = j.dst; st.src_len = j.src_len; st.dst_cap = j.dst_cap;
        st.format = j.format; st.image = j.image;
        const int64_t cb = c->cfg[SPNG_CFG_BLOCK_CUT_BYTES];
        const uint64_t cut_bytes = cb == 0 ? RESUME_SERIAL_BITS / 8 : (uint64_t)cb;
        uint64_t origin = 0;
        bool cut = p.internal && cb != SPNG_BLOCK_CUT_NEVER && j.src_len >= cut_bytes;
        if (!p.internal && cb != SPNG_BLOCK_CUT_NEVER) {
            const uint64_t *s4 = &p.state[4 * i];
            const uint64_t at = (s4[2] ? s4[2] : s4[0]) / 8;
            if ((s4[0] | s4[1] | s4[2] | s4[3]) && j.src_len >= at && j.src_len - at >= cut_bytes) {
                cut = true; st.cut_resumed = 1;
                origin = at & ~(uint64_t)255;
            }
        }
        if (!p.state.empty()) {
            st.start_bit = p.state[4 * i]; st.out_pos = p.state[4 * i + 1]; st.blk_out = st.out_pos;
            if (st.cut_resumed && p.state[4 * i + 2]) { st.tok_bit = p.state[4 * i + 2]; st.out_pos = p.state[4 * i + 3]; }
            if (!p.internal && !st.cut_resumed && p.state[4 * i + 2] && p.state[4 * i + 2] - p.state[4 * i] > RESUME_SERIAL_BITS) st.serial_only = 1;
        }
        st.seg_first = (uint32_t)p.segs.size();
        st.seg_origin = origin;
        const uint64_t span = j.src_len - origin;
        uint64_t k = (span + seg_bytes - 1) / seg_bytes;
        if (k < 1) k = 1;
        if (p.segs.size() + k > 0x7fffffffu) return SPNG_E_ARGUMENT;
        st.seg_count = (uint32_t)k; st.seg_bytes = seg_bytes;
        if (cut) {
            const uint64_t cs = st.cut_resumed ? cut_bytes / seg_bytes : (cut_bytes + seg_bytes - 1) / seg_bytes;
            st.cut_segs = (uint32_t)(cs > 0x7fffffffu ? 0x7fffffffu : cs < 1 ? 1 : cs);
            p.cuts = true;
        }
        for (uint64_t q = 0; q < k; ++q) {
            PSeg sg;
            memset(&sg, 0, sizeof sg);
            sg.stream = (uint32_t)i; sg.index = (uint32_t)q;
            const uint64_t len = q + 1 < k ? seg_bytes : span - q * seg_bytes;
            uint64_t most = 16 * len;
            if (most > 2 * (j.dst_cap + 64)) most = 2 * (j.dst_cap + 64);
            sg.log_cap = (most >> 16) + 2;
            sg.log_off = log; log += sg.log_cap;
            sg.start_bit = ~0ull;
            p.segs.push_back(sg);
        }
        uint64_t e = (uint64_t)(per_byte * (double)span);
        if (e > 2 * (j.dst_cap + 64)) e = 2 * (j.dst_cap + 64);
        p.est[i] = e + k * 65536 + 65536;
        if (st.cut_segs && !(c->block_bytes > 0 && c->block_bytes < 262144)) p.est[i] += k * 65536;
    }
    p.log_bytes = log * 4;
    return SPNG_DONE;
}

static int32_t size_token_pool(spng_ctx *c, InflatePlan &p)
{
    if (int32_t st = c->grow(c->d_log, c->log_cap, p.log_bytes, p.log_bytes / 8)) return st;
    uint64_t want = 0, largest = 0;
    for (auto e : p.est) { want += e; if (e > largest) largest = e; }
    uint64_t budget = (uint64_t)c->cfg[SPNG_CFG_TOKEN_BYTES];
    if (!budget) {
        size_t free_b = 0, total_b = 0;
        HIP_TRY(hipMemGetInfo(&free_b, &total_b));
        budget = (uint64_t)(free_b + c->tok_cap) / 2;
        if (budget < (64ull << 20)) budget = 64ull << 20;
    }
    if (budget < 2 * largest && !c->cfg[SPNG_CFG_TOKEN_BYTES]) budget = 2 * largest;
    uint64_t need = want < budget ? want : budget;
    if (need < largest) need = largest;
    need = (need + 65535) & ~(uint64_t)65535;
    bool failed = false;
    if (int32_t st = c->grow(c->d_tok, c->tok_cap, need, 0, &failed)) return st;
    if (failed) {
        p.parallel = false; p.streams.clear(); p.segs.clear();
    }
    return SPNG_DONE;
}

static void group_streams(const spng_ctx *c, InflatePlan &p)
{
    uint64_t want = 0, largest = 0;
    for (auto e : p.est) { want += e; if (e > largest) largest = e; }
    const uint64_t pool = c->tok_cap & ~(uint64_t)65535;
    p.pool_pages = (uint32_t)(pool >> 16 > 0xfffffff0ull ? 0xfffffff0ull : pool >> 16);
    uint64_t share = pool;
    if (want > pool) {
        const uint64_t ng = (want + pool - 1) / pool;
// ... 25 lines not shown
        if (c->cfg[SPNG_CFG_RESOLVE_PARTS] <= 1) {
            uint64_t most = 0;
            for (auto &j : p.jobs) most = j.dst_cap > most ? j.dst_cap : most;
            const uint64_t by_size = most >> 20 < 2 ? 2 : most >> 20;
            if (pm > by_size) pm = (uint32_t)by_size;
        }
        uint64_t syms = 0;
        for (size_t i = 0; i < p.jobs.size(); ++i) {
            p.streams[i].sym_off = syms;
            syms += (p.jobs[i].dst_cap + 15) & ~(uint64_t)7;
        }
        const uint64_t win = (uint64_t)p.jobs.size() * pm * 32768;
        bool afford = syms * 2 <= c->sym_cap;
        if (!afford && !(c->sym_failed && syms * 2 >= c->sym_failed)) {
            size_t free_b = 0, total_b = 0;
            HIP_TRY(hipMemGetInfo(&free_b, &total_b));
            afford = syms * 2 + win <= (uint64_t)(free_b + c->sym_cap + c->win_cap) / 4;
        }
        if (pm >= 2 && afford) {
            bool failed = false;
            if (syms * 2 > c->sym_cap) {
                if (int32_t st = c->grow(c->d_sym, c->sym_cap, syms * 2, 0, &failed)) return st;
                c->sym_failed = failed ? syms * 2 : 0;
            }
            if (!failed)
                if (int32_t st = c->grow(c->d_win, c->win_cap, win, 0, &failed)) return st;
            if (!failed) {
                p.pmax = pm;
                for (auto &st : p.streams) st.parts_max = pm;
            }
        }
    }
    if (!p.pmax && c->d_sym && p.jobs.size() > 384) {
        HIP_TRY(hipStreamSynchronize(c->stream));
        HIP_TRY(hipFree(c->d_sym)); c->d_sym = nullptr; c->sym_cap = 0;
    }
    return SPNG_DONE;
}

static int32_t plan_inflate(spng_ctx *c, InflatePlan &p)
{
    p.internal = p.state.empty();
    if (p.internal) p.state.assign(p.jobs.size() * 4, 0);
    for (auto &j : p.jobs) j.internal = p.internal ? 1 : 0;
    p.parallel = c->cfg[SPNG_CFG_INFLATE_MODE] != SPNG_INFLATE_SERIAL && !p.jobs.empty();
    for (auto &j : p.jobs) p.gzip = p.gzip || j.format == SPNG_FORMAT_GZIP;
    if (!p.parallel) return SPNG_DONE;
    uint64_t total = 0;
    for (auto &j : p.jobs) total += j.src_len;
    if (int32_t st = learn_from_last_batch(c, total)) return st;
    if (int32_t st = cut_into_segments(c, p, inflate_segment_bytes((uint64_t)c->cfg[SPNG_CFG_SEGMENT_BYTES], total, c->block_bytes))) return st;
    if (int32_t st = size_token_pool(c, p)) return st;
    if (!p.parallel) return SPNG_DONE;
    group_streams(c, p);
    if (int32_t st = plan_parts(c, p)) return st;
    c->pool_pages_planned = p.pool_pages;
    c->pool_src_bytes = total;
    if (!c->h_pool_used) {
        HIP_TRY(hipHostMalloc((void **)&c->h_pool_used, 64, hipHostMallocDefault));
        HIP_TRY(hipEventCreateWithFlags(&c->pool_ev, hipEventDisableTiming));
    }
    return SPNG_DONE;
}

static void stage_inflate(InflatePlan &p, Arena &a)
{
    const size_t n = p.jobs.size();
    p.jobs_at = a.take(n * sizeof(InflateJob));
    if (!p.state.empty()) {
        p.state_at = a.take(n * 32);
        memcpy(a.host<uint64_t>(p.state_at), p.state.data(), n * 32);
        for (size_t i = 0; i < n; ++i) {
            p.jobs[i].state = a.dev<uint64_t>(p.state_at) + 4 * i;
            if (p.parallel) p.streams[i].state = p.jobs[i].state;
        }
    }
    if (p.parallel) {
        p.streams_at = a.take(n * sizeof(PStream));
        p.segs_at = a.take(p.segs.size() * sizeof(PSeg));
        memcpy(a.host<PStream>(p.streams_at), p.streams.data(), n * sizeof(PStream));
        memcpy(a.host<PSeg>(p.segs_at), p.segs.data(), p.segs.size() * sizeof(PSeg));
    }
    if (p.parallel) {
        p.next_at = a.take(64);
        memset(a.host<uint32_t>(p.next_at), 0, 64);
        if (p.pmax) {
            p.parts_at = a.take(n * p.pmax * sizeof(PPart));
            memset(a.host<PPart>(p.parts_at), 0, n * p.pmax * sizeof(PPart));
        }
    }
    if (p.parallel || p.gzip) {
        p.done_at = a.take(n * 4);
        memset(a.host<int32_t>(p.done_at), 0, n * 4);
        for (size_t i = 0; i < n; ++i) p.jobs[i].skip = a.dev<int32_t>(p.done_at) + i;
    }
    memcpy(a.host<InflateJob>(p.jobs_at), p.jobs.data(), n * sizeof(InflateJob));
}

static int32_t trace_inflate_plan(spng_ctx *c, const InflatePlan &p, Arena &a)
{
    const uint32_t n = (uint32_t)p.jobs.size();
    std::vector<PStream> hs(n);
    std::vector<PSeg> hg(p.segs.size());
    HIP_TRY(hipStreamSynchronize(c->stream));
    HIP_TRY(hipMemcpy(hs.data(), a.dev<PStream>(p.streams_at), n * sizeof(PStream), hipMemcpyDeviceToHost));
    HIP_TRY(hipMemcpy(hg.data(), a.dev<PSeg>(p.segs_at), hg.size() * sizeof(PSeg), hipMemcpyDeviceToHost));
    {
        uint64_t nostart = 0, fail = 0, skipped = 0; uint32_t shown = 0;
        for (uint32_t i = 0; i < n; ++i) {
            const PStream &st = hs[i];
            for (uint32_t k = 0; k < st.seg_count; ++k) {
                const PSeg &sg = hg[st.seg_first + k];
                const bool a = sg.start_bit == ~0ull, b = !a && sg.status != PSEG_CONT && sg.status != PSEG_FINAL, cskip = !a && !b && sg.status == PSEG_CONT && sg.next != k + 1;
                nostart += a; fail += b; skipped += cskip;
                if ((a || b || cskip) && shown < 12) {
                    ++shown;
                    fprintf(stderr, "[pinflate] anomaly: stream %u seg %u/%u start %lld end %lld status %d next %u ntok %llu\n", i, k, st.seg_count,
                            (long long)sg.start_bit, (long long)sg.end_bit, sg.status, sg.next, (unsigned long long)sg.ntok);
                }
            }
        }
        fprintf(stderr, "[pinflate] %u streams, %zu segments in %zu groups, pool %u pages: %llu without a start, %llu failed, %llu ran past the next start\n", n,
                hg.size(), p.groups.size(), p.pool_pages, (unsigned long long)nostart, (unsigned long long)fail, (unsigned long long)skipped);
    }
    for (uint32_t i = 0; i < n && i < 4; ++i) {
        const PStream &st = hs[i];
        fprintf(stderr, "[pinflate] stream %u: len %llu segs %u seg_bytes %llu ok %d pass %u ntok %llu end_bit %llu\n", i,
                (unsigned long long)st.src_len, st.seg_count, (unsigned long long)st.seg_bytes, st.ok, st.pass,
                (unsigned long long)st.ntok, (unsigned long long)st.end_bit);
        for (uint32_t k = 0; k < st.seg_count && k < 12; ++k) {
            const PSeg &sg = hg[st.seg_first + k];
            fprintf(stderr, "   seg %u: start %lld end %lld status %d used %u ntok %llu tok_base %llu next %u", k,
                    (long long)sg.start_bit, (long long)sg.end_bit, sg.status, sg.used, (unsigned long long)sg.ntok,
                    (unsigned long long)sg.tok_base, sg.next);
            if (sg.head) fprintf(stderr, " head %u", sg.head);
            fprintf(stderr, "\n");
        }
    }
    return SPNG_DONE;
}

static int32_t launch_inflate_plan(spng_ctx *c, InflatePlan &p, Arena &a, spng_result *dr)
{
    const uint32_t n = (uint32_t)p.jobs.size();
    if (p.gzip)
        HIP_TRY(launch_gzip_pre(a.dev<InflateJob>(p.jobs_at), p.parallel ? a.dev<PStream>(p.streams_at) : nullptr, dr,
                                a.dev<uint64_t>(p.gz_at), a.dev<int32_t>(p.done_at), n, c->stream));
    if (p.parallel) {
        Timed whole(c, SPNG_K_PINFLATE);
        PStream *ds = a.dev<PStream>(p.streams_at);
        PSeg *dg = a.dev<PSeg>(p.segs_at);
        int32_t *dd = a.dev<int32_t>(p.done_at);
        uint32_t *dnext = a.dev<uint32_t>(p.next_at);
        uint32_t *dlog = (uint32_t *)c->d_log;
        uint8_t *pool = (uint8_t *)c->d_tok;
        const uint32_t pages = p.pool_pages;
        const hipStream_t q = c->stream;
        c->cut_stats_valid = false;
        for (size_t gi = 0; gi <= p.groups.size(); ++gi) {
            const bool retry = gi == p.groups.size();
            const InflatePlan::Group g = retry ? InflatePlan::Group{0, n, 0, (uint32_t)p.segs.size()} : p.groups[gi];
            if (gi) HIP_TRY(hipMemsetAsync(dnext, 0, 4, q));
            { Timed t(c, SPNG_K_PINF_FIND, q); HIP_TRY(launch_pinf2_find(ds, dg, g.g0, g.g1 - g.g0, retry, q)); }
            bool cuts = false;
            if (!retry) for (uint32_t i = g.s0; i < g.s1 && !cuts; ++i) cuts = p.streams[i].cut_segs != 0;
            PCut *dc = p.cuts ? a.dev<PCut>(p.cuts_at) : nullptr;
            if (cuts) {
                c->cut_stats_valid = true;
                Timed t(c, SPNG_K_PINF_DECODE, q);
                HIP_TRY(hipMemsetAsync(dc + g.g0, 0, (size_t)(g.g1 - g.g0) * sizeof(PCut), q));
                HIP_TRY(launch_pinf2_cutplan(ds + g.s0, g.s1 - g.s0, dg, dc, dnext + 12, q));
                HIP_TRY(launch_pinf2_cutdecode(ds, dg, dc, g.g0, g.g1 - g.g0, dlog, pool, dnext, pages, q));
                HIP_TRY(launch_pinf2_cutjoin(ds, dg, dc, g.g0, g.g1 - g.g0, dlog, pool, dnext, pages, dnext + 12, q));
            } else
            { Timed t(c, SPNG_K_PINF_DECODE, q); HIP_TRY(launch_pinf2_decode(ds, dg, g.g0, g.g1 - g.g0, dlog, pool, dnext, pages, retry, q)); }
            PPart *dparts = p.pmax ? a.dev<PPart>(p.parts_at) + (size_t)g.s0 * p.pmax : nullptr;
            const uint32_t pm = retry ? 0u : p.pmax;
            if (cuts) HIP_TRY(launch_pinf2_cutscan(ds + g.s0, g.s1 - g.s0, dg, dc, dparts, dnext + 12, q));
            else HIP_TRY(launch_pinf2_scan(ds + g.s0, g.s1 - g.s0, dg, dparts, retry, q));
            {
                Timed t(c, SPNG_K_PINF_RESOLVE, q);
                if (pm) {
                    if (int32_t st = second_stream(c)) return st;
                    HIP_TRY(hipEventRecord(c->ev_fork, q));
                    HIP_TRY(hipStreamWaitEvent(c->stream2, c->ev_fork, 0));
                    HIP_TRY(launch_pinf2_parts(ds + g.s0, g.s1 - g.s0, dg, dlog, pool, pages, dr, dd + g.s0, dparts, pm, (uint16_t *)c->d_sym, c->stream2));
                }
                HIP_TRY(launch_pinf2_resolve(ds + g.s0, g.s1 - g.s0, dg, dlog, pool, pages, dr, dd + g.s0, dparts, pm, retry, q));
                if (pm) {
                    HIP_TRY(hipEventRecord(c->ev_join, c->stream2));
                    HIP_TRY(hipStreamWaitEvent(q, c->ev_join, 0));
                    HIP_TRY(launch_pinf2_join(ds + g.s0, g.s1 - g.s0, dr, dd + g.s0, dparts, pm, (uint16_t *)c->d_sym,
                                              (uint8_t *)c->d_win + (size_t)g.s0 * pm * 32768, q));
                }
            }
            HIP_TRY(launch_pinf2_account(dnext, dnext + 8, pages, q));
        }
        if (c->cut_stats_valid) HIP_TRY(hipMemcpyAsync(c->h_pool_used + 8, dnext + 12, 12, hipMemcpyDeviceToHost, c->stream));
        if (!c->pool_pending) {
            HIP_TRY(hipMemcpyAsync(c->h_pool_used, dnext + 8, 16, hipMemcpyDeviceToHost, c->stream));
            c->pool_src_pending = c->pool_src_bytes;
            HIP_TRY(hipEventRecord(c->pool_ev, c->stream));
            c->pool_pending = true;
        }
    }
    if (p.parallel && getenv("SPNG_TRACE_PINFLATE"))
        if (int32_t st = trace_inflate_plan(c, p, a)) return st;
    {
        Timed t(c, SPNG_K_INFLATE);
        HIP_TRY(launch_inflate(a.dev<InflateJob>(p.jobs_at), n, dr, c->stream));
    }
    if (p.gzip)
        HIP_TRY(launch_gzip_inflate_post(a.dev<InflateJob>(p.jobs_at), dr, a.dev<uint64_t>(p.gz_at), a.dev<uint32_t>(p.gzparts_at), n,
                                         c->stream));
    if (!p.state.empty())
        HIP_TRY(launch_resume_post(a.dev<InflateJob>(p.jobs_at), dr, a.dev<uint64_t>(p.sumparts_at), n, c->stream));
    return SPNG_DONE;
}

static const uint64_t *rows_len_in_results(void *user, uint32_t i)
{
    return &((spng_result *)user)[i].written;
}
static const uint64_t *rows_len_in_array(void *user, uint32_t i)
{
    return user ? (const uint64_t *)user + i : nullptr;
}

}

extern "C" {

static int32_t inflate_batch(spng_ctx *c, const spng_stream_desc *descs, const uint64_t *h_state, bool resume, uint32_t count,
                             spng_result *d_results, spng_result *h_results)
{
    if (!c || (!descs && count) || (!d_results && !h_results && count)) return SPNG_E_ARGUMENT;
    if (!count) return SPNG_DONE;
    HIP_TRY(hipSetDevice(c->device));
    std::lock_guard<std::mutex> g(c->mu);
    InflatePlan plan;
    plan.jobs.resize(count);
    if (resume) plan.state.assign((size_t)count * 4, 0);
    for (uint32_t i = 0; i < count; ++i) {
        if ((!descs[i].d_src && descs[i].src_len) || (!descs[i].d_dst && descs[i].dst_cap) || descs[i].format < SPNG_FORMAT_ZLIB ||
            descs[i].format > SPNG_FORMAT_GZIP) return SPNG_E_ARGUMENT;
        plan.jobs[i] = InflateJob{(const uint8_t *)descs[i].d_src, (uint8_t *)descs[i].d_dst,
                                  descs[i].src_len, descs[i].dst_cap, descs[i].format, i, nullptr, nullptr, 0, 0};
        if (resume && h_state) {
            const uint64_t *hs = h_state + 4 * (size_t)i;
            for (int k = 0; k < 4; ++k) plan.state[4 * (size_t)i + k] = hs[k];
            if (hs[0] > descs[i].src_len * 8 || hs[1] > descs[i].dst_cap || hs[2] > descs[i].src_len * 8 || hs[3] > descs[i].dst_cap ||
                (hs[2] && (hs[2] <= hs[0] || hs[3] < hs[1])) || (!hs[2] && hs[3])) return SPNG_E_ARGUMENT;
        }
    }
    if (int32_t st = plan_inflate(c, plan)) return st;
    if (int32_t st = c->reserve(plan.bytes() + count * sizeof(spng_result) + 1024)) return st;
    Arena a{c};
    stage_inflate(plan, a);
    const size_t upload = a.off;
    const size_t res = a.take(count * sizeof(spng_result));
    if (plan.gzip) { plan.gz_at = a.take(count * 8); plan.gzparts_at = a.take((size_t)count * 4 * gzip_pieces()); }
    plan.sumparts_at = a.take((size_t)count * 8 * gzip_pieces());
    plan.take_cuts(a);
    if (int32_t st = c->upload(0, upload)) return st;
    spng_result *dr = d_results ? d_results : a.dev<spng_result>(res);
    poison_results_kernel<<<(count + 255) / 256, 256, 0, c->stream>>>(dr, count);
    HIP_TRY(hipGetLastError());
    if (int32_t st = launch_inflate_plan(c, plan, a, dr)) return st;
    return read_back(c, h_results, dr, count * sizeof(spng_result));
}

int32_t spng_inflate_batch(spng_ctx *c, const spng_stream_desc *descs, uint32_t count,
                           spng_result *d_results, spng_result *h_results)
{
    return inflate_batch(c, descs, nullptr, false, count, d_results, h_results);
}

int32_t spng_inflate_resume_batch(spng_ctx *c, const spng_stream_desc *descs, const uint64_t *h_state, uint32_t count,
                                  spng_result *d_results, spng_result *h_results)
{
    return inflate_batch(c, descs, h_state, true, count, d_results, h_results);
// ... 316 lines not shown
```

### swift_png_amd/csrc/pinflate2.hip

```cpp
#include "common.hpp"
#include <type_traits>
#include <cstddef>
#include "huffman.hpp"

namespace spng {

#ifdef SPNG_EMU
#define AS_GLOBAL
#else
#define AS_GLOBAL __attribute__((address_space(1)))
#endif
__device__ __forceinline__ uint32_t mul24(uint32_t a, uint32_t b)
{
#ifdef SPNG_EMU
    return (a & 0xffffffu) * (b & 0xffffffu);
#else
    uint32_t r;
    asm("v_mul_u32_u24 %0, %1, %2" : "=v"(r) : "v"(a), "v"(b));
    return r;
#endif
}
typedef uint32_t v4u __attribute__((vector_size(16)));
struct __attribute__((packed)) PV4 { v4u v; };
typedef uint8_t AS_GLOBAL g8;
typedef uint16_t AS_GLOBAL g16;
typedef uint32_t AS_GLOBAL g32;
typedef PV4 AS_GLOBAL gPV4;
typedef uint32_t v2u __attribute__((vector_size(8)));
struct __attribute__((packed)) PV2 { v2u v; };
typedef PV2 AS_GLOBAL gPV2;

#ifdef SPNG_NO_HINTS
#define RARE(c) (c)
#else
#define RARE(c) __builtin_expect((c), 0)
#endif
static constexpr int LB = 9, DB = 8, MB = 7;
#ifndef SPNG_SDW_MAX
#define SPNG_SDW_MAX 9
#endif
static constexpr int SDW_MAX = SPNG_SDW_MAX;
static constexpr int STAGE2_DW = SDW_MAX * 64 + 16;
static constexpr uint32_t PAGE_SHIFT = 16;
static constexpr uint32_t PAGE_UNITS = 1u << (PAGE_SHIFT - 4);
static constexpr uint64_t NONE2 = ~0ull;
static constexpr uint32_t TK_NULL = 0xffffu;

__device__ __forceinline__ uint32_t tk_m0(uint32_t run, uint32_t dist) { return 0x8000u | ((dist - 1) & 63) << 8 | (run - 3); }
__device__ __forceinline__ uint32_t tk_m1(uint32_t dist) { return 0xC000u | (dist - 1) >> 6; }

struct DPool { uint8_t *base; uint32_t *next; uint32_t pages, pad; };

#ifdef SPNG_D_PROF
#define DP_ARG , uint64_t *dp
#define DP_PASS , dp
#define DP(k) do { const uint64_t now_ = __builtin_readcyclecounter(); dp[k] += now_ - dp[31]; dp[31] = now_; } while (0)
#define DPN(k, v) (dp[k] += (v))
#define HP_ARG , uint64_t *dp = nullptr
#define HP(k) do { if (dp) DP(k); } while (0)
#else
#define DP_ARG
#define DP_PASS
#define DP(k)
#define DPN(k, v)
#define HP_ARG
#define HP(k)
#endif

#if defined(SPNG_EMU) && defined(SPNG_EMU_COV)
static long g_cov[13];
#define COV(k) __atomic_fetch_add(&g_cov[k], 1, __ATOMIC_RELAXED)
#else
#define COV(k) ((void)0)
#endif

static constexpr uint32_t EXT = 480;

enum { C_LIT = 0, C_EOB = 1, C_REF = 2, C_BAD = 3, C_LIT2 = 6, C_LINK = 7 };
__device__ __forceinline__ uint32_t lit_entry2(uint32_t sym, uint32_t len)
{
    if (sym < 256) return len | C_LIT << 5 | len << 8 | sym << 16;
    if (sym == 256) return len | C_EOB << 5 | len << 8;
    uint32_t base, cx;
    if (sym < 265) { base = sym - 254; cx = 0; }
    else if (sym < 285) { cx = (sym - 261) >> 2; base = ((4 + ((sym - 265) & 3)) << cx) + 3; }
    else if (sym == 285) { base = 258; cx = 0; }
    else { base = 0; cx = 0; }
    return (len + cx) | (base ? C_REF : C_BAD) << 5 | len << 8 | cx << 12 | base << 16;
}
__device__ __forceinline__ uint32_t dist_entry2(uint32_t sym, uint32_t len)
{
    uint32_t base, ox;
    if (sym < 4) { base = sym + 1; ox = 0; }
    else if (sym < 30) { ox = (sym >> 1) - 1; base = ((2 + (sym & 1)) << ox) + 1; }
    else { base = 0; ox = 0; }
    return (len + ox) | (base ? 0u : 32u) | len << 8 | ox << 12 | base << 16;
}
static constexpr uint32_t DIST_UNDEF = 1 | 32;

struct DLds {
    uint32_t lit[1 << LB];
    uint32_t dist[1 << DB];
    uint32_t ext[EXT];
    uint32_t stage[STAGE2_DW];
    union {
        struct {
            uint8_t  lens[512];
            uint32_t clut[1 << MB];
            uint32_t hb[6][16];
            uint32_t cl[32];
            uint16_t first[2][16];
            uint16_t codes[6][64];
        } h;
        struct {
            uint32_t ent[64];
            uint32_t vmap[SDW_MAX * 64];
            uint16_t flag[64], mpos[64];
        } c;
    };
};
static constexpr uint32_t QB = (uint32_t)offsetof(DLds, stage) * 8;
static_assert(QB % 32 == 0 && QB + (SDW_MAX * 64 + 3) * 32 + 64 < 65536, "biased positions: dword-aligned, 16 bits");
static_assert(offsetof(DLds, c.vmap) == offsetof(DLds, c.ent) + 256 && offsetof(DLds, c.flag) == offsetof(DLds, c.vmap) + SDW_MAX * 256,
              "round 1 reads ent as the row in front of vmap; round 0's empty OR behind a lane's last word lands in flag / mpos");

__device__ __forceinline__ v4u ld16(const g8 *src, uint64_t n, uint64_t off)
{
    v4u v = {0, 0, 0, 0};
    if (off + 16 <= n) v = ((const gPV4 *)(src + off))->v;
    else if (off < n) {
        uint32_t w[4] = {0, 0, 0, 0};
        for (int b = 0; b < 16; ++b) if (off + b < n) w[b >> 2] |= (uint32_t)src[off + b] << (8 * (b & 3));
        v[0] = w[0]; v[1] = w[1]; v[2] = w[2]; v[3] = w[3];
    }
    return v;
}
__device__ __forceinline__ void stage_bytes2(uint32_t *dst, const g8 *src, uint64_t n, uint64_t from, int dwords, int lane)
{
    for (int k = 0; k * 256 < dwords; ++k)
        if (k * 256 + lane * 4 < dwords) *(v4u *)(dst + k * 256 + lane * 4) = ld16(src, n, from + (uint64_t)k * 1024 + (uint64_t)lane * 16);
    WSYNC();
}
__device__ __forceinline__ void fetch2(const uint32_t *stage, uint32_t q, uint32_t &lo, uint32_t &hi)
{
    const uint32_t w = q >> 5;
    const uint32_t d0 = stage[w], d1 = stage[w + 1], d2 = stage[w + 2];
    lo = __builtin_amdgcn_alignbit(d1, d0, q);
    hi = __builtin_amdgcn_alignbit(d2, d1, q);
}
__device__ __forceinline__ uint32_t upeek32_2(const uint32_t *stage, uint32_t q)
{
    uint32_t lo, hi;
    fetch2(stage, q, lo, hi);
// ... 998 lines not shown
            const uint32_t a = cuts[first + i].anchor;
            if (a != ~0u) {
                const uint64_t lo = org + (uint64_t)(a + 1) * sb, hi = org + (uint64_t)nf * sb < n ? org + (uint64_t)nf * sb : n;
                const uint64_t b = segs[first + a].start_bit;
                const uint64_t from = a == 0 && rcut ? org : lo;
                if (hi > lo && hi - from >= (uint64_t)need * sb && b + 3 <= n * 8) {
                    const uint32_t v = (uint32_t)src[b >> 3] | ((b >> 3) + 1 < n ? (uint32_t)src[(b >> 3) + 1] << 8 : 0u);
                    const uint32_t type = (v >> ((b & 7) + 1)) & 3;
                    cut = type == 1 || type == 2;
                }
            }
            cuts[first + i].cut = cut ? 1u : 0u;
        }
        tried += (uint32_t)__popcll(__ballot(cut));
        if (mask) nxt = base + (uint32_t)__ffsll((long long)mask) - 1;
        if (base == 0) break;
    }
    if (lane == 0 && tried) { atomicAdd(stats, tried); st.cut_on = 1; }
    if (!tried && uni64(st.tok_bit)) back_to_the_header(st, segs, lane);
}

__global__ __launch_bounds__(64, SPNG_D_WAVES) void pinf2_cutjoin_kernel(const PStream *__restrict__ streams, PSeg *__restrict__ segs,
                                                                        PCut *__restrict__ cuts, uint32_t *__restrict__ pt_slab, DPool pool, uint32_t seg0,
                                                                        uint32_t *__restrict__ stats)
{
    __shared__ __attribute__((aligned(16))) DLds s;
    const int lane = threadIdx.x;
    const PSeg &pd = segs[seg0 + blockIdx.x];
    PCut &pc = cuts[seg0 + blockIdx.x];
    if ((int32_t)UNI(pd.status) != PSEG_CUT) return;
    const PStream &st = streams[UNI(pd.stream)];
    const uint32_t j = UNI(pd.next);
    if (j <= UNI(pd.index) || j >= UNI(st.seg_count)) return;
    const PCut &sg = cuts[UNI(st.seg_first) + j];
    const uint32_t nrec = UNI(sg.nrec);
    if (!UNI(sg.cut) || !nrec) return;
    const g8 *src = (const g8 *)uni64((uint64_t)st.src);
    const uint64_t n = uni64(st.src_len);
    const uint64_t want = uni64(sg.head_tbl);
    uint64_t pos = uni64(pd.end_bit), id = uni64(pc.tbl_id);
    g32 *pt = (g32 *)(pt_slab + uni64(pd.log_off));
    const uint32_t pt_cap = uni64(pd.log_cap) > 0xffffff00ull ? 0xffffff00u : (uint32_t)uni64(pd.log_cap);
    Cursor cur;
    cur.nhw = uni64(pd.ntok); cur.npages = (uint32_t)((cur.nhw + PAGE_HW - 1) >> (PAGE_SHIFT - 1)); cur.dry = false;
    cur.pa = (cur.nhw & (PAGE_HW - 1)) ? (g8 *)(pool.base + ((uint64_t)UNI(pt[cur.nhw >> (PAGE_SHIFT - 1)]) << PAGE_SHIFT)) : nullptr;
    const uint64_t hw0 = cur.nhw;
    uint64_t nbytes = 0;
    uint32_t c = 0, chunks = 0;
    bool mid = true, have = false, ok = false;
    uint64_t jt = 0, jt_bytes = 0;
    Hdr2 h;
    for (uint32_t steps = 0; steps < 4 * CUT_JOIN_CHUNKS; ++steps) {
        while (c < nrec && uni64(sg.rec[c].bit) < pos) ++c;
        if (c == nrec) break;
        if (mid && uni64(sg.rec[c].bit) == pos) { ok = id == want; break; }
        if (chunks == CUT_JOIN_CHUNKS) break;
        if (!have || !mid) {
            const uint64_t at = mid ? uni64(pc.tbl) : pos;
            if (!UB(parse_header2(s, src, n, at, h, lane)) || h.type == 0) break;
            have = true;
            if (!mid) { id = table_id(h, pos); jt = pos; jt_bytes = nbytes; pos = h.payload; mid = true; continue; }
        }
        const uint32_t sdw = chunk_dwords(h.minlen);
        const uint64_t chb = (uint64_t)sdw * 32 * 64, upto = uni64(sg.rec[c].bit);
        uint64_t next;
        const uint32_t state = cut_chunk<true>(s, h, src, n, pos, pos, sdw, pool, pt, pt_cap, cur, next, nbytes, upto - pos < chb ? upto : pos + chb, lane);
        chunks += 1;
        if (state == 2) break;
        pos = uni64(next);
        if (state == 1) { if (h.bfinal) break; mid = false; }
    }
    if (!ok) return;
    if (chunks > 1) COV(7);
    if (lane == 0) {
        pc.add_tok = cur.nhw - hw0; pc.add_bytes = nbytes;
        pc.next_head = UNI(sg.rec[c].hw); pc.next_sub = UNI(sg.rec[c].bytes); pc.joined = 1;
        pc.next_bit = pos; pc.join_tbl = jt; pc.join_tbl_bytes = jt_bytes;
        atomicAdd(stats + 1, 1u);
    }
}

template <uint32_t RETRY, bool CUT>
__device__ __forceinline__ void scan_stream(PStream *__restrict__ streams, PSeg *__restrict__ segs, PPart *__restrict__ parts, uint32_t *__restrict__ stats,
                                            const PCut *__restrict__ cuts)
{
    constexpr uint32_t retry = RETRY;
    const int lane = threadIdx.x;
    PStream &st = streams[blockIdx.x];
    if (retry && UNI(st.pass) != 1) {
        if (lane == 0) st.ok = 0;
        return;
    }
    const uint32_t first = UNI(st.seg_first), count = UNI(st.seg_count);
    bool ok = false, partial = false, dry = false;
    uint64_t tok = 0, end_bit = 0, out = 0;
    uint32_t k = 0;
    bool met_cut = false, by_cut = false;
    uint32_t skip_hw = 0; uint64_t skip_bytes = 0;
    const bool rcut = CUT && UNI(st.cut_resumed) != 0;
    uint64_t cur_hdr = CUT ? uni64(st.start_bit) : 0, cur_out = CUT ? uni64(st.blk_out) : 0, ho_bit = 0;
    bool handed = false;
    for (uint32_t hops = 0; hops < count; ++hops) {
        PSeg *sg = segs + first + k;
        const uint64_t start = uni64(sg->start_bit), end = uni64(sg->end_bit);
        const int32_t status = (int32_t)UNI(sg->status);
        if (status == PSEG_NOPAGE && (start != NONE2 || (CUT && by_cut))) dry = true;
        if ((start == NONE2 && !(CUT && by_cut)) || status == PSEG_FAIL || status == PSEG_NOPAGE) break;
        if constexpr (CUT) {
            uint64_t nt = uni64(sg->ntok), nb = uni64(sg->nbytes);
            const uint32_t hd = by_cut ? skip_hw : 0u;
            if (by_cut) nb -= skip_bytes;
            uint32_t nx = 0;
            if (status == PSEG_CUT) {
                met_cut = true;
                nx = UNI(sg->next);
                const PCut &ct = cuts[first + k];
                const bool joined = nx > k && nx < count && UNI(cuts[first + nx].cut) && UNI(ct.joined);
                if (rcut) {
                    if (UNI(ct.tbl_here)) { cur_hdr = uni64(ct.tbl); cur_out = uni64(st.out_pos) + out + uni64(ct.tbl_bytes) - (by_cut ? skip_bytes : 0); }
                    if (!joined || (int32_t)UNI(segs[first + nx].status) == PSEG_FAIL) {
                        ho_bit = end;
                        if (joined) {
                            if (uni64(ct.join_tbl)) { cur_hdr = uni64(ct.join_tbl); cur_out = uni64(st.out_pos) + out + nb + uni64(ct.join_tbl_bytes); }
                            nt += uni64(ct.add_tok); nb += uni64(ct.add_bytes); ho_bit = uni64(ct.next_bit);
                        }
                        if (lane == 0) { sg->tok_base = tok; sg->out_base = out; sg->used = 1; sg->ntok = nt; sg->nbytes = nb; sg->head = hd; sg->status = PSEG_PARTIAL; }
                        tok += nt - hd; out += nb;
                        handed = true;
                        break;
                    }
                    if (uni64(ct.join_tbl)) { cur_hdr = uni64(ct.join_tbl); cur_out = uni64(st.out_pos) + out + nb + uni64(ct.join_tbl_bytes); }
                }
                if (!joined) break;
                nt += uni64(ct.add_tok); nb += uni64(ct.add_bytes);
                skip_hw = UNI(ct.next_head); skip_bytes = uni64(ct.next_sub);
            }
            if (lane == 0) { sg->tok_base = tok; sg->out_base = out; sg->used = 1; sg->ntok = nt; sg->nbytes = nb; sg->head = hd; }
            tok += nt - hd;
            out += nb;
            if (status == PSEG_CUT) { k = nx; by_cut = true; continue; }
            by_cut = false;
        } else {
        if (lane == 0) { sg->tok_base = tok; sg->out_base = out; sg->used = 1; }
        tok += uni64(sg->ntok);
        out += uni64(sg->nbytes);
        }
        if (status == PSEG_FINAL) { ok = true; end_bit = end; break; }
        if (status == PSEG_PARTIAL) { ok = true; partial = true; end_bit = end; break; }
        const uint32_t nx = UNI(sg->next);
        if (nx <= k || nx >= count) break;
        if (uni64(segs[first + nx].start_bit) != end) break;
        k = nx;
    }
    if (CUT && handed && uni64(st.src_len) * 8 - ho_bit <= 2 * uni64(st.seg_bytes) * 8) { ok = true; partial = true; end_bit = ho_bit; }
    else handed = false;
    if (CUT && met_cut && !(ok && (!partial || rcut))) {
        ok = false; partial = false; dry = true; handed = false;
        if (lane == 0) atomicAdd(stats + 2, 1u);
        COV(8);
    }
    bool again = !retry && dry;
    if constexpr (CUT) { if (again && uni64(st.tok_bit)) again = back_to_the_header(st, segs, lane); }
    const uint32_t pmax = UNI(st.parts_max);
    uint32_t np = 0;
    if (pmax > 1 && ok && uni64(st.start_bit) == 0 && uni64(st.out_pos) == 0 && out <= uni64(st.dst_cap) && out > 0) {
        PPart *pp = parts + (uint64_t)blockIdx.x * pmax;
        uint64_t w0 = (uint64_t)gridDim.x * (pmax - 1) > 256 ? 1 : 0;
#ifdef SPNG_EMU
        if (getenv("EMU_FIRST_PART_SHARE")) w0 = 1;
#endif
        uint64_t begun = 0;
        uint32_t kk = 0, tnext = 1;
        np = 1;
        if (lane == 0) { pp[0].seg = 0; pp[0].out_pos = 0; pp[0].present = 1; }
        for (uint32_t hops = 0; hops < count; ++hops) {
            const PSeg *sg = segs + first + kk;
            const uint64_t ob = uni64(sg->out_base);
            if (kk != 0 && tnext < pmax && ob >= 32768u && ob > begun && ob * (2 * pmax + w0) >= (uint64_t)(2 * tnext + w0) * out) {
                if (lane == 0) {
                    pp[np].seg = kk; pp[np].out_pos = ob; pp[np].present = 1;
                    pp[np - 1].seg_end = kk; pp[np - 1].out_len = ob - begun;
                }
                begun = ob; np += 1;
                tnext = (uint32_t)((ob * (2 * pmax + w0) / out + 2 - w0) / 2);
            }
            if ((int32_t)UNI(sg->status) == PSEG_FINAL || (int32_t)UNI(sg->status) == PSEG_PARTIAL) break;
            kk = UNI(sg->next);
        }
        if (lane == 0) { pp[np - 1].seg_end = ~0u; pp[np - 1].out_len = out - begun; }
    }
    if (lane == 0) { st.ok = ok ? (handed ? 3 : partial ? 2 : 1) : 0; st.ntok = tok; st.end_bit = end_bit; st.pass = again ? 1 : 0; st.tok_base = 0;
                     st.out_total = out; st.parts = np; st.ho_hdr = cur_hdr; st.ho_out = cur_out; }
}

template <uint32_t RETRY>
__global__ __launch_bounds__(64) void pinf2_scan_kernel(PStream *__restrict__ streams, PSeg *__restrict__ segs, PPart *__restrict__ parts)
{
    scan_stream<RETRY, false>(streams, segs, parts, nullptr, nullptr);
}
__global__ __launch_bounds__(64) void pinf2_cutscan_kernel(PStream *__restrict__ streams, PSeg *__restrict__ segs, const PCut *__restrict__ cuts,
                                                           PPart *__restrict__ parts, uint32_t *__restrict__ stats)
{
    scan_stream<0, true>(streams, segs, parts, stats, cuts);
}

#ifndef SPNG_R_THREADS
#define SPNG_R_THREADS 512
#define SPNG_R_WAVES 4
#endif
static constexpr uint32_t RT2 = SPNG_R_THREADS;
static constexpr uint32_t NW2 = RT2 / 64;
template <bool BIG> struct RGeo {
    static constexpr uint32_t TILE = BIG ? 8192 : 4096;
    static constexpr uint32_t BPT = TILE / RT2;
    static constexpr uint32_t HPT = TILE / 2 / RT2;
    static constexpr uint32_t EB = BPT < 8 ? BPT : 8;
    static constexpr uint32_t MAXM = TILE / 8;
};
static constexpr uint32_t WINDOW2 = 32768;
static constexpr uint32_t R2_DONE = 0x8000;
static constexpr uint32_t PTC = 256;

template <bool MARK> struct RingOf { typedef uint8_t T; };
template <> struct RingOf<true> { typedef uint16_t T; };
template <bool MARK, bool BIG>
struct RLds2T {
    typename RingOf<MARK>::T ring[WINDOW2];
    uint16_t state[RGeo<BIG>::TILE];
    uint32_t rec[RGeo<BIG>::MAXM + 2][2];
    uint32_t bitmap[RGeo<BIG>::TILE / 32];
    uint16_t h0[RT2 + 8];
    uint32_t pt[PTC];
    uint32_t part[3 * NW2];
    uint32_t cut[2];
};

template <class L>
__device__ __forceinline__ uint32_t block_excl_scan2(L &s, uint32_t v, uint32_t &total, int tid)
{
    const int lane = tid & 63, wave = tid >> 6;
    uint32_t wt;
    const uint32_t off = wave_excl_scan(v, wt, lane);
    if (lane == 0) s.part[wave] = wt;
    __syncthreads();
    uint32_t before = 0, all = 0;
#pragma unroll
    for (int w4 = 0; w4 < (int)NW2; w4 += 4) {
        const v4u p = *(const v4u *)(s.part + w4);
#pragma unroll
        for (int c = 0; c < 4; ++c) { before += w4 + c < wave ? p[c] : 0u; all += p[c]; }
    }
    total = all;
    return off + before;
}

__device__ __forceinline__ void stream_verdict(const PStream &st, uint32_t S, uint32_t I, uint64_t pos, spng_result *__restrict__ results,
                                               int32_t *__restrict__ done)
{
    const g8 *src = (const g8 *)st.src;
    const uint64_t n = st.src_len;
    uint64_t *state = st.state;
    const bool whole = st.start_bit == 0 && st.out_pos == 0;
    if (st.ok == 2 || st.ok == 3) {
        const bool tok = st.ok == 3;
        state[0] = tok ? st.ho_hdr : st.end_bit; state[1] = tok ? st.ho_out : pos; state[2] = tok ? st.end_bit : 0; state[3] = tok ? pos : 0;
    } else if (!whole) {
        const uint64_t endb = (st.end_bit + 7) / 8, consumed = endb + (st.format == SPNG_FORMAT_ZLIB ? 4 : 0);
        spng_result &res = results[st.image];
        if (consumed <= n) {
            res.status = SPNG_DONE; res.reserved = 1;
            res.written = pos; res.consumed = consumed;
            res.aux[0] = res.aux[1] = 0;
            *done = 1;
        }
    } else {
        const uint64_t endb = (st.end_bit + 7) / 8;
        spng_result &res = results[st.image];
        if (st.format == SPNG_FORMAT_IOS) {
            res.status = SPNG_DONE; res.reserved = 1;
            res.written = pos; res.consumed = endb;
            res.aux[0] = res.aux[1] = 0;
            *done = 1;
        } else if (endb + 4 <= n) {
            const uint32_t declared = (uint32_t)src[endb] << 24 | (uint32_t)src[endb + 1] << 16 |
                                      (uint32_t)src[endb + 2] << 8 | (uint32_t)src[endb + 3];
            const uint32_t N = (uint32_t)(pos % 65521);
            const uint32_t computed = (uint32_t)((N + (uint64_t)N * S % 65521 + 65521 - I) % 65521) << 16 | (1 + S) % 65521;
            res.status = declared == computed ? SPNG_DONE : SPNG_E_STREAM_CHECKSUM; res.reserved = 1;
            res.written = pos; res.consumed = endb + 4;
            res.aux[0] = declared == computed ? 0 : declared; res.aux[1] = declared == computed ? 0 : computed;
            *done = 1;
        }
    }
}

template <uint32_t RETRY, bool MARK, bool BIG>
__global__ __launch_bounds__(RT2, SPNG_R_WAVES) void pinf2_resolve_kernel(const PStream *__restrict__ streams, const PSeg *__restrict__ segs,
                                                               const uint32_t *__restrict__ pt_slab, DPool pool,
                                                               spng_result *__restrict__ results, int32_t *__restrict__ done,
                                                               PPart *__restrict__ parts, uint32_t pmax, uint16_t *__restrict__ sym)
{
    constexpr uint32_t retry = RETRY;
    constexpr uint32_t TILE2 = RGeo<BIG>::TILE, BPT2 = RGeo<BIG>::BPT, HPT2 = RGeo<BIG>::HPT, EB2 = RGeo<BIG>::EB, MAXM2 = RGeo<BIG>::MAXM;
    static_assert(HPT2 == 8 || HPT2 == 4, "a thread's halfwords of a window are one 16- or 8-byte load");
    constexpr uint32_t DONE = MARK ? 0x4000u : R2_DONE;
    constexpr uint32_t KNOWN = MARK ? 0xc000u : R2_DONE;
    __shared__ __attribute__((aligned(16))) RLds2T<MARK, BIG> s;
    const int tid = threadIdx.x, lane = tid & 63, wave = (int)UNI((uint32_t)tid >> 6);
    const uint32_t sidx = MARK ? blockIdx.x / (pmax - 1) : blockIdx.x;
    const uint32_t pidx = MARK ? 1 + blockIdx.x % (pmax - 1) : 0;
    const PStream &st = streams[sidx];
    if (!UNI(st.ok) || (retry && done[sidx])) return;
    const uint32_t nparts = pmax ? UNI(st.parts) : 0;
    if (MARK && pidx >= nparts) return;
    PPart *part = nparts > 1 ? parts + (uint64_t)sidx * pmax + pidx : nullptr;
    const uint32_t seg_end = part ? UNI(part->seg_end) : ~0u;
    const uint64_t part_pos = part ? uni64(part->out_pos) : 0;
    g8 *dst = (g8 *)uni64((uint64_t)st.dst);
    const uint64_t cap = uni64(st.dst_cap);
    uint64_t pos = uni64(st.out_pos) + part_pos;
    uint32_t accS = 0, accI = 0;
    uint32_t pmod = (uint32_t)(pos % 65521);
    bool bad = false, over = false;
    g16 *symo = MARK ? (g16 *)(sym + uni64(st.sym_off)) : nullptr;
    if (!MARK && pos) {
        for (uint64_t p = (pos > WINDOW2 ? pos - WINDOW2 : 0) + (uint32_t)tid; p < pos; p += RT2) s.ring[p & (WINDOW2 - 1)] = dst[p];
    }
    if (tid < (int)(TILE2 / 32)) s.bitmap[tid] = 0;
    if (tid == 0) { s.rec[0][0] = 0; s.rec[0][1] = 1; }
    __syncthreads();
    const uint32_t seg_first = UNI(st.seg_first), seg_count = UNI(st.seg_count);
    uint32_t sk = part ? UNI(part->seg) : 0;
#ifdef SPNG_D_PROF
    uint64_t rp[12] = {0, 0, 0, 0, 0, 0, 0, 0, 0, 0, 0, 0}, rp_t = __builtin_readcyclecounter();
#define RP2(k) do { const uint64_t now_ = __builtin_readcyclecounter(); rp[k] += now_ - rp_t; rp_t = now_; } while (0)
#define RPN2(k, v) (rp[k] += (v))
#else
#define RP2(k)
#define RPN2(k, v)
#endif
    constexpr uint32_t NULL2 = TK_NULL | TK_NULL << 16;
    for (uint32_t hops = 0; hops < seg_count && !over && sk != seg_end; ++hops) {
        const PSeg &sg = segs[seg_first + sk];
        const uint64_t nhw = uni64(sg.ntok);
        const g32 *ptg = (const g32 *)(pt_slab + uni64(sg.log_off));
        const int32_t sstatus = (int32_t)UNI(sg.status);
        uint64_t cursor = UNI(sg.head);
        uint64_t pt_lo = 0;
        __syncthreads();
        for (uint32_t i = (uint32_t)tid; i < PTC; i += RT2) s.pt[i] = (pt_lo + i) * PAGE_UNITS * 8 < nhw + 8 ? ptg[pt_lo + i] : 0u;
        __syncthreads();
        uint32_t tv[HPT2 / 2];
        auto load_window = [&](uint64_t from) {
            const uint64_t h = (from & ~(uint64_t)(HPT2 - 1)) + (uint64_t)tid * HPT2;
#pragma unroll
            for (int k = 0; k < (int)(HPT2 / 2); ++k) tv[k] = NULL2;
            if (h < nhw) {
                const uint64_t u = h >> 3;
                const uint32_t pid = s.pt[(u >> (PAGE_SHIFT - 4)) - pt_lo];
                const g8 *q = (const g8 *)pool.base + ((uint64_t)pid << PAGE_SHIFT) + ((u & (PAGE_UNITS - 1)) << 4) + ((h & 7) << 1);
                if constexpr (HPT2 == 8) { const v4u v = ((const gPV4 *)q)->v; tv[0] = v[0]; tv[1] = v[1]; tv[2] = v[2]; tv[3] = v[3]; }
                else { const v2u v = ((const gPV2 *)q)->v; tv[0] = v[0]; tv[1] = v[1]; }
            }
        };
        load_window(cursor);
        while (cursor < nhw) {
            RP2(0);
            const uint64_t wb = cursor;
            uint32_t hh[HPT2];
#pragma unroll
            for (int j = 0; j < (int)HPT2; ++j) {
                const uint32_t idx = (uint32_t)tid * HPT2 + j;
                const uint32_t v = (tv[j >> 1] >> (16 * (j & 1))) & 0xffff;
                hh[j] = wb + idx < nhw ? v : TK_NULL;
            }
            s.h0[tid] = (uint16_t)hh[0];
            if (tid == 0) s.cut[1] = 0xffffffffu;
            uint32_t bytes = 0, refs = 0;
#pragma unroll
            for (int j = 0; j < (int)HPT2; ++j) {
                const uint32_t v = hh[j];
                const bool lit = !(v & 0x8000), m0 = (v & 0xC000) == 0x8000;
                bytes += lit ? 1u : m0 ? (v & 0xff) + 3 : 0u;
                refs += m0 ? 1u : 0u;
            }
            uint32_t total;
            const uint32_t offp = block_excl_scan2(s, refs << 20 | bytes, total, tid);
            RP2(1);
            uint32_t curb = offp & 0xfffff, curm = offp >> 20;
            const uint32_t hnext = tid + 1 < (int)RT2 ? s.h0[tid + 1] : TK_NULL;
            const bool front = curb <= TILE2 && curm <= MAXM2;
            const bool fits = curb + bytes <= TILE2 && curm + refs <= MAXM2 &&
                              !(tid == (int)RT2 - 1 && (hh[HPT2 - 1] & 0xC000) == 0x8000);
            if (front && !fits) { s.cut[0] = curb; s.cut[1] = (uint32_t)tid * HPT2; if (curb + bytes <= TILE2 && curm + refs > MAXM2) COV(9); }
            if (fits) {
#pragma unroll
                for (int j = 0; j < (int)HPT2; ++j) {
                    const uint32_t v = hh[j];
                    if (!(v & 0x8000)) { s.state[curb] = (uint16_t)(DONE | v); curb += 1; }
                    else if ((v & 0xC000) == 0x8000) {
                        const uint32_t len = (v & 0xff) + 3;
                        const uint32_t h1 = j < (int)HPT2 - 1 ? hh[j < (int)HPT2 - 1 ? j + 1 : (int)HPT2 - 1] : hnext;
                        const uint32_t dd = (((v >> 8) & 63) | (h1 & 0x1ff) << 6) + 1;
                        atomicOr(&s.bitmap[curb >> 5], 1u << (curb & 31));
                        s.rec[curm + 1][0] = curb | len << 16;
                        s.rec[curm + 1][1] = dd;
                        curb += len; curm += 1;
                    }
                }
            }
            __syncthreads();
            const uint32_t cut0 = s.cut[0], cut1 = s.cut[1];
            const uint64_t wend = nhw - wb < (uint64_t)RT2 * HPT2 ? nhw - wb : (uint64_t)RT2 * HPT2;
            const uint32_t tlen = cut1 != 0xffffffffu ? cut0 : total & 0xfffff;
            const uint32_t wlast = cut1 != 0xffffffffu ? cut1 : (uint32_t)wend;
            if (pos + tlen > cap) { over = true; break; }
            const uint64_t cursor_next = wb + wlast;
            if ((((cursor_next + 2 * RT2 * HPT2) >> 3) >> (PAGE_SHIFT - 4)) >= pt_lo + PTC) {
                __syncthreads();
                pt_lo = (cursor_next >> 3) >> (PAGE_SHIFT - 4);
                for (uint32_t i = (uint32_t)tid; i < PTC; i += RT2) s.pt[i] = (pt_lo + i) * PAGE_UNITS * 8 < nhw + 8 ? ptg[pt_lo + i] : 0u;
                __syncthreads();
            }
            load_window(cursor_next);
            RP2(2);
            const uint32_t rbase = (uint32_t)pos & (WINDOW2 - 1);
            const bool early = pos - part_pos < WINDOW2;
            uint32_t sv[BPT2];
            {
                v4u bw = {0, 0, 0, 0};
                if ((uint32_t)lane < TILE2 / 128) bw = *(const v4u *)(s.bitmap + 4 * lane);
                const uint32_t ca = (uint32_t)__popc(bw[0]) + (uint32_t)__popc(bw[1]), cbb = (uint32_t)__popc(bw[2]) + (uint32_t)__popc(bw[3]);
                uint32_t tt;
                const uint32_t rb = wave_excl_scan(ca + cbb, tt, lane);
                const bool odd = wave & 1;
                const uint32_t srclo = odd ? bw[2] : bw[0], srchi = odd ? bw[3] : bw[1], srcbase = odd ? rb + ca : rb;
                auto expand_rows = [&](auto early_c) {
                constexpr bool EARLY = decltype(early_c)::value;
#pragma unroll
                for (int part = 0; part < (int)(BPT2 / EB2); ++part) {
                    v2u recv[EB2];
#pragma unroll
                    for (int kk = 0; kk < (int)EB2; ++kk) {
                        const int k = part * (int)EB2 + kk;
                        const uint32_t row = (uint32_t)wave + NW2 * k;
                        const uint32_t mlo = (uint32_t)__builtin_amdgcn_readlane((int)srclo, (int)(row >> 1));
                        const uint32_t mhi = (uint32_t)__builtin_amdgcn_readlane((int)srchi, (int)(row >> 1));
                        const uint32_t base = (uint32_t)__builtin_amdgcn_readlane((int)srcbase, (int)(row >> 1));
                        const unsigned long long mw1 = ((unsigned long long)mhi << 32 | mlo) >> 1;
                        const uint32_t id = __builtin_amdgcn_mbcnt_hi((uint32_t)(mw1 >> 32), __builtin_amdgcn_mbcnt_lo((uint32_t)mw1, base + (mlo & 1)));
                        recv[kk] = *(const v2u *)s.rec[id];
                    }
                    uint32_t siv[EB2], farv[EB2];
#pragma unroll
                    for (int kk = 0; kk < (int)EB2; ++kk) {
                        const int k = part * (int)EB2 + kk;
                        const uint32_t j = ((uint32_t)wave + NW2 * k) * 64 + (uint32_t)lane;
                        const uint32_t startb = recv[kk][0] & 0xffff, len = recv[kk][0] >> 16, d = recv[kk][1];
                        uint32_t kk2 = j - startb;
                        const bool inside = kk2 < len;
                        if (inside && kk2 >= d) COV(10);
                        if (inside && kk2 >= d) kk2 -= mul24(d, (uint32_t)(((float)kk2 + 0.5f) * __builtin_amdgcn_rcpf((float)d)));
                        if (inside && kk2 >= d) COV(12);
                        siv[kk] = inside ? startb - d + kk2 : 0x7fffffffu;
                        farv[kk] = s.ring[(rbase + siv[kk]) & (WINDOW2 - 1)];
                    }
#pragma unroll
                    for (int kk = 0; kk < (int)EB2; ++kk) {
                        const int k = part * (int)EB2 + kk;
                        const uint32_t j = ((uint32_t)wave + NW2 * k) * 64 + (uint32_t)lane;
                        const uint32_t si = siv[kk];
                        sv[k] = DONE;
                        if (si != 0x7fffffffu) {
                            uint32_t v;
                            if (MARK) {
                                const uint32_t rel = (uint32_t)(pos - part_pos) + si;
                                v = (int32_t)si >= 0 ? si : (!EARLY || (int32_t)rel >= 0) ? farv[kk] : 0x8000u | (rel + WINDOW2);
                                if (EARLY && (int32_t)si < 0 && (int32_t)rel < 0) COV(11);
                            } else {
                                if (EARLY && (int32_t)si < 0 && (uint32_t)pos < 0u - si) bad = true;
                                v = (int32_t)si < 0 ? DONE | farv[kk] : si;
                            }
                            sv[k] = v;
                            s.state[j] = (uint16_t)v;
                        }
                    }
                }
                };
                if (early) expand_rows(std::true_type{}); else expand_rows(std::false_type{});
            }
            __syncthreads();
            RP2(3);
            if (tid < (int)(TILE2 / 32)) s.bitmap[tid] = 0;
            for (;;) {
                asm volatile("" ::: "memory");
                bool more = false;
                uint32_t gv[BPT2];
#pragma unroll
                for (int k = 0; k < (int)BPT2; ++k) { gv[k] = DONE; if (!(sv[k] & KNOWN)) gv[k] = s.state[sv[k]]; }
#pragma unroll
                for (int k = 0; k < (int)BPT2; ++k) {
                    if (!(sv[k] & KNOWN)) {
// ... 9 lines not shown
            {
                uint32_t bv[BPT2];
#pragma unroll
                for (int k = 0; k < (int)BPT2; ++k) bv[k] = s.state[((uint32_t)wave + NW2 * k) * 64 + (uint32_t)lane];
#pragma unroll
                for (int k = 0; k < (int)BPT2; ++k) {
                    const uint32_t j = ((uint32_t)wave + NW2 * k) * 64 + (uint32_t)lane;
                    if (j < tlen) s.ring[(rbase + j) & (WINDOW2 - 1)] = (typename RingOf<MARK>::T)bv[k];
                }
            }
            __syncthreads();
            if constexpr (MARK) {
                const uint64_t u0 = pos >> 3, u1 = (pos + tlen) >> 3;
                for (uint64_t u = u0 + (uint32_t)tid; u < u1; u += RT2) {
                    const uint16_t *r = s.ring + ((u << 3) & (WINDOW2 - 1));
                    if ((u << 3) >= part_pos) ((gPV4 *)(symo + (u << 3)))->v = *(const v4u *)r;
                    else for (int c = 0; c < 8; ++c) if ((u << 3) + c >= part_pos) symo[(u << 3) + c] = r[c];
                }
            } else {
                const uint64_t u0 = pos >> 4, u1 = (pos + tlen) >> 4;
                for (uint64_t u = u0 + (uint32_t)tid; u < u1; u += RT2) {
                    const v4u v = *(const v4u *)(s.ring + ((u << 4) & (WINDOW2 - 1)));
                    ((gPV4 *)(dst + (u << 4)))->v = v;
                    uint32_t A = 0, J = 0;
                    A = __builtin_amdgcn_sad_u8(v[0], 0, A); A = __builtin_amdgcn_sad_u8(v[1], 0, A);
                    A = __builtin_amdgcn_sad_u8(v[2], 0, A); A = __builtin_amdgcn_sad_u8(v[3], 0, A);
                    J = __builtin_amdgcn_udot4(v[0], 0x03020100u, J, false);
                    J = __builtin_amdgcn_udot4(v[1], 0x07060504u, J, false);
                    J = __builtin_amdgcn_udot4(v[2], 0x0b0a0908u, J, false);
                    J = __builtin_amdgcn_udot4(v[3], 0x0f0e0d0cu, J, false);
                    const uint32_t g = (pmod + 65521u - ((uint32_t)pos & 15u) + 16u * (uint32_t)(u - u0)) % 65521u;
                    accS = (accS + A) % 65521u;
                    accI = (accI + g * A + J) % 65521u;
                }
            }
            pos += tlen;
            pmod = (pmod + tlen) % 65521u;
            cursor = cursor_next;
            RP2(5);
            RPN2(8, 1); RPN2(10, tlen);
        }
        if (sstatus == PSEG_FINAL || sstatus == PSEG_PARTIAL) break;
        sk = UNI(sg.next);
    }
#ifdef SPNG_D_PROF
    if (blockIdx.x == 0 && (tid == 0 || tid == 300))
        printf("resolve[t%d]: %lu tiles (%lu bytes), %lu rounds; cycles: loop %lu window+scan %lu take+prefetch %lu expand %lu jump %lu store %lu\n",
               tid, rp[8], rp[10], rp[9], rp[0], rp[1], rp[2], rp[3], rp[4], rp[5]);
#endif
    __syncthreads();
    if constexpr (MARK) {
        const uint64_t u1 = pos >> 3 << 3, at = u1 + (uint32_t)tid;
        if (!over && at < pos && at >= part_pos) symo[at] = s.ring[at & (WINDOW2 - 1)];
    } else {
        const uint64_t u1 = pos >> 4 << 4;
        if (!over && u1 + (uint32_t)tid < pos) {
            const uint32_t b = s.ring[(u1 + (uint32_t)tid) & (WINDOW2 - 1)];
            dst[u1 + (uint32_t)tid] = (uint8_t)b;
            const uint32_t g = (uint32_t)((u1 + (uint32_t)tid) % 65521);
            accS = (accS + b) % 65521;
            accI = (uint32_t)((accI + (uint64_t)g * b) % 65521);
        }
    }
    if (__syncthreads_or(bad || over)) {
        if (part && tid == 0) part->failed = 1;
        return;
    }
    if constexpr (MARK) return;
    else {
        const uint32_t S1 = wave_sum(accS) % 65521, I1 = wave_sum(accI % 65521) % 65521;
        __syncthreads();
        if (lane == 0) { s.part[wave] = S1; s.part[NW2 + wave] = I1; }
        __syncthreads();
        uint32_t S = 0, I = 0;
        for (int w = 0; w < (int)NW2; ++w) { S += s.part[w]; I += s.part[NW2 + w]; }
        S %= 65521; I %= 65521;
        if (part) {
            if (tid == 0) { part->sumS = S; part->sumI = I; }
            return;
        }
        if (tid == 0) stream_verdict(st, S, I, pos, results, done + sidx);
    }
}

__global__ __launch_bounds__(512) void pinf2_window_kernel(const PStream *__restrict__ streams, const PPart *__restrict__ parts, uint32_t pmax,
                                                           const uint16_t *__restrict__ sym, uint8_t *__restrict__ win)
{
    const PStream &st = streams[blockIdx.x];
    const uint32_t np = UNI(st.parts);
    if (!UNI(st.ok) || np < 2) return;
    const PPart *pp = parts + (uint64_t)blockIdx.x * pmax;
    const g8 *dst = (const g8 *)uni64((uint64_t)st.dst);
    const g16 *symo = (const g16 *)(sym + uni64(st.sym_off));
    g8 *w = (g8 *)win + (uint64_t)blockIdx.x * pmax * WINDOW2;
    for (uint32_t p = 1; p < np; ++p) {
        const uint64_t from = uni64(pp[p].out_pos) - WINDOW2, before = uni64(pp[p - 1].out_pos);
        for (uint32_t o = threadIdx.x; o < WINDOW2; o += 512) {
            const uint64_t a = from + o;
            uint32_t b;
            if (p == 1) b = dst[a];
            else if (a >= before) {
                const uint32_t v = symo[a];
                b = v & 0x8000 ? w[(uint64_t)(p - 1) * WINDOW2 + (v & 0x7fff)] : v & 0xff;
            } else b = w[(uint64_t)(p - 1) * WINDOW2 + (uint32_t)(a - (before - WINDOW2))];
            w[(uint64_t)p * WINDOW2 + o] = (uint8_t)b;
        }
        __threadfence();
        __syncthreads();
    }
}

static constexpr uint32_t FIX_WG = 32;
__global__ __launch_bounds__(256) void pinf2_fixup_kernel(const PStream *__restrict__ streams, PPart *__restrict__ parts, uint32_t pmax,
                                                          const uint16_t *__restrict__ sym, const uint8_t *__restrict__ win)
{
    const uint32_t sidx = blockIdx.y / (pmax - 1), pidx = 1 + blockIdx.y % (pmax - 1);
    const PStream &st = streams[sidx];
    if (!UNI(st.ok) || pidx >= UNI(st.parts)) return;
    PPart &part = parts[(uint64_t)sidx * pmax + pidx];
    if (UNI(part.failed)) return;
    const uint64_t p0 = uni64(part.out_pos), p1 = p0 + uni64(part.out_len);
    g8 *dst = (g8 *)uni64((uint64_t)st.dst);
    const g16 *symo = (const g16 *)(sym + uni64(st.sym_off));
    const g8 *w = (const g8 *)win + ((uint64_t)sidx * pmax + pidx) * WINDOW2;
    unsigned long long S = 0, I = 0;
    const uint64_t u0 = p0 >> 3, u1 = (p1 + 7) >> 3;
    for (uint64_t u = u0 + (uint64_t)blockIdx.x * 256 + threadIdx.x; u < u1; u += (uint64_t)FIX_WG * 256) {
        const uint64_t at = u << 3;
        const bool inner = at >= p0 && at + 8 <= p1;
        uint32_t b[8];
        if (inner) {
            const v4u v = ((const gPV4 *)(symo + at))->v;
#pragma unroll
            for (int c = 0; c < 8; ++c) b[c] = (v[c >> 1] >> (16 * (c & 1))) & 0xffff;
        } else {
#pragma unroll
            for (int c = 0; c < 8; ++c) b[c] = (at + c >= p0 && at + c < p1) ? (uint32_t)symo[at + c] : 0x4000u;
        }
#pragma unroll
        for (int c = 0; c < 8; ++c) b[c] = b[c] & 0x8000 ? (uint32_t)w[b[c] & 0x7fff] : b[c] & 0xff;
        if (inner) {
            v2u o;
            o[0] = b[0] | b[1] << 8 | b[2] << 16 | b[3] << 24; o[1] = b[4] | b[5] << 8 | b[6] << 16 | b[7] << 24;
            ((gPV2 *)(dst + at))->v = o;
        } else {
#pragma unroll
            for (int c = 0; c < 8; ++c) if (at + c >= p0 && at + c < p1) dst[at + c] = (uint8_t)b[c];
        }
        const uint32_t g = (uint32_t)(at % 65521);
#pragma unroll
        for (int c = 0; c < 8; ++c) {
            const bool mine = inner || (at + c >= p0 && at + c < p1);
            const uint32_t v = mine ? b[c] : 0u;
            S += v; I += (unsigned long long)((g + (uint32_t)c) % 65521u) * v;
        }
    }
#pragma unroll
    for (int m = 32; m >= 1; m >>= 1) {
        S += (unsigned long long)(uint32_t)__shfl_xor((int)(uint32_t)S, m, 64) | (unsigned long long)(uint32_t)__shfl_xor((int)(uint32_t)(S >> 32), m, 64) << 32;
        I += (unsigned long long)(uint32_t)__shfl_xor((int)(uint32_t)I, m, 64) | (unsigned long long)(uint32_t)__shfl_xor((int)(uint32_t)(I >> 32), m, 64) << 32;
    }
    if ((threadIdx.x & 63) == 0) { atomicAdd(&part.sumS, S); atomicAdd(&part.sumI, I); }
}

__global__ void pinf2_verdict_kernel(const PStream *__restrict__ streams, const PPart *__restrict__ parts, uint32_t pmax,
                                     spng_result *__restrict__ results, int32_t *__restrict__ done, uint32_t count)
{
    const uint32_t i = blockIdx.x * blockDim.x + threadIdx.x;
    if (i >= count) return;
    const PStream &st = streams[i];
    if (!st.ok || st.parts < 2 || done[i]) return;
    const PPart *pp = parts + (uint64_t)i * pmax;
    unsigned long long S = 0, I = 0;
    for (uint32_t p = 0; p < st.parts; ++p) {
        if (pp[p].failed) return;
        S = (S + pp[p].sumS % 65521) % 65521; I = (I + pp[p].sumI % 65521) % 65521;
    }
    stream_verdict(st, (uint32_t)S, (uint32_t)I, st.out_total, results, done + i);
}

__global__ void pinf2_account_kernel(uint32_t *ctr, uint32_t *totals, uint32_t pages)
{
    const uint32_t used = ctr[0];
    atomicAdd(&totals[0], used < pages ? used : pages);
    if (used >= pages) atomicOr(&totals[1], 1u);
    atomicAdd(&totals[2], ctr[1]); ctr[1] = 0;
}

#ifndef SPNG_EMU
hipError_t launch_pinf2_find(PStream *d_streams, PSeg *d_segs, uint32_t seg0, uint32_t nsegs, uint32_t retry, hipStream_t stream)
{
    if (retry) pinf2_find_kernel<1><<<nsegs, 64, 0, stream>>>(d_streams, d_segs, seg0);
    else pinf2_find_kernel<0><<<nsegs, 64, 0, stream>>>(d_streams, d_segs, seg0);
    return hipGetLastError();
}
hipError_t launch_pinf2_decode(PStream *d_streams, PSeg *d_segs, uint32_t seg0, uint32_t nsegs, uint32_t *d_pt, uint8_t *d_pool, uint32_t *d_next,
                               uint32_t pages, uint32_t retry, hipStream_t stream)
{
    DPool pool{d_pool, d_next, pages, 0};
    if (retry) pinf2_decode_kernel<1><<<nsegs, 64, 0, stream>>>(d_streams, d_segs, d_pt, pool, seg0);
    else pinf2_decode_kernel<0><<<nsegs, 64, 0, stream>>>(d_streams, d_segs, d_pt, pool, seg0);
    return hipGetLastError();
}
hipError_t launch_pinf2_cutplan(PStream *d_streams, uint32_t nstreams, PSeg *d_segs, PCut *d_cuts, uint32_t *d_stats, hipStream_t stream)
{
    pinf2_cutplan_kernel<<<nstreams, 64, 0, stream>>>(d_streams, d_segs, d_cuts, d_stats);
    return hipGetLastError();
}
hipError_t launch_pinf2_cutdecode(PStream *d_streams, PSeg *d_segs, PCut *d_cuts, uint32_t seg0, uint32_t nsegs, uint32_t *d_pt, uint8_t *d_pool,
                                  uint32_t *d_next, uint32_t pages, hipStream_t stream)
{
    DPool pool{d_pool, d_next, pages, 0};
    pinf2_cutdecode_kernel<1><<<nsegs, 64, 0, stream>>>(d_streams, d_segs, d_pt, pool, seg0, d_cuts);
    pinf2_cutdecode_kernel<2><<<nsegs, 64, 0, stream>>>(d_streams, d_segs, d_pt, pool, seg0, d_cuts);
    return hipGetLastError();
}
hipError_t launch_pinf2_cutjoin(PStream *d_streams, PSeg *d_segs, PCut *d_cuts, uint32_t seg0, uint32_t nsegs, uint32_t *d_pt, uint8_t *d_pool,
                                uint32_t *d_next, uint32_t pages, uint32_t *d_stats, hipStream_t stream)
{
    DPool pool{d_pool, d_next, pages, 0};
    pinf2_cutjoin_kernel<<<nsegs, 64, 0, stream>>>(d_streams, d_segs, d_cuts, d_pt, pool, seg0, d_stats);
    return hipGetLastError();
}
hipError_t launch_pinf2_cutscan(PStream *d_streams, uint32_t nstreams, PSeg *d_segs, PCut *d_cuts, PPart *d_parts, uint32_t *d_stats, hipStream_t stream)
{
    pinf2_cutscan_kernel<<<nstreams, 64, 0, stream>>>(d_streams, d_segs, d_cuts, d_parts, d_stats);
    return hipGetLastError();
}
hipError_t launch_pinf2_scan(PStream *d_streams, uint32_t nstreams, PSeg *d_segs, PPart *d_parts, uint32_t retry, hipStream_t stream)
{
    if (retry) pinf2_scan_kernel<1><<<nstreams, 64, 0, stream>>>(d_streams, d_segs, d_parts);
    else pinf2_scan_kernel<0><<<nstreams, 64, 0, stream>>>(d_streams, d_segs, d_parts);
    return hipGetLastError();
}
hipError_t launch_pinf2_resolve(PStream *d_streams, uint32_t nstreams, PSeg *d_segs, uint32_t *d_pt, uint8_t *d_pool, uint32_t pages,
                                spng_result *d_results, int32_t *d_done, PPart *d_parts, uint32_t pmax, uint32_t retry, hipStream_t stream)
{
    DPool pool{d_pool, nullptr, pages, 0};
    if (retry) pinf2_resolve_kernel<1, false, true><<<nstreams, RT2, 0, stream>>>(d_streams, d_segs, d_pt, pool, d_results, d_done, d_parts, pmax, nullptr);
    else pinf2_resolve_kernel<0, false, true><<<nstreams, RT2, 0, stream>>>(d_streams, d_segs, d_pt, pool, d_results, d_done, d_parts, pmax, nullptr);
    return hipGetLastError();
}
hipError_t launch_pinf2_parts(PStream *d_streams, uint32_t nstreams, PSeg *d_segs, uint32_t *d_pt, uint8_t *d_pool, uint32_t pages,
                              spng_result *d_results, int32_t *d_done, PPart *d_parts, uint32_t pmax, uint16_t *d_sym, hipStream_t stream)
{
    DPool pool{d_pool, nullptr, pages, 0};
    if (nstreams * (pmax - 1) > 256) pinf2_resolve_kernel<0, true, false><<<nstreams * (pmax - 1), RT2, 0, stream>>>(d_streams, d_segs, d_pt, pool, d_results, d_done, d_parts, pmax, d_sym);
    else pinf2_resolve_kernel<0, true, true><<<nstreams * (pmax - 1), RT2, 0, stream>>>(d_streams, d_segs, d_pt, pool, d_results, d_done, d_parts, pmax, d_sym);
    return hipGetLastError();
}
hipError_t launch_pinf2_join(PStream *d_streams, uint32_t nstreams, spng_result *d_results, int32_t *d_done, PPart *d_parts, uint32_t pmax,
                             uint16_t *d_sym, uint8_t *d_win, hipStream_t stream)
{
    pinf2_window_kernel<<<nstreams, 512, 0, stream>>>(d_streams, d_parts, pmax, d_sym, d_win);
    pinf2_fixup_kernel<<<dim3(FIX_WG, nstreams * (pmax - 1)), 256, 0, stream>>>(d_streams, d_parts, pmax, d_sym, d_win);
    pinf2_verdict_kernel<<<(nstreams + 63) / 64, 64, 0, stream>>>(d_streams, d_parts, pmax, d_results, d_done, nstreams);
    return hipGetLastError();
}
hipError_t launch_pinf2_account(uint32_t *d_ctr, uint32_t *d_totals, uint32_t pages, hipStream_t stream)
{
    pinf2_account_kernel<<<1, 1, 0, stream>>>(d_ctr, d_totals, pages);
    return hipGetLastError();
}
#endif

}
```

Measured before the change: 35820.

## Classify streams by token density and resolve dense ones with a wide-window kernel

The scan pass now labels each stream narrow or wide from its token-to-output ratio and counts both classes. By default two resolve kernels are launched: the existing one, and a variant that reads twice as many halfwords per thread per window step. Each kernel presumably skips streams of the other class. The aim is to cut per-step overhead for token-dense streams, at the cost of an extra kernel launch and another stats copy to the host on every batch.

```diff
diff --git a/include/spng_mi355.h b/include/spng_mi355.h
--- a/include/spng_mi355.h
+++ b/include/spng_mi355.h
@@ -109,8 +109,10 @@
        SPNG_CFG_DEFLATE_BYTES = 7,
        SPNG_CFG_MULTI_GROUPS = 8,
        SPNG_CFG_BLOCK_CUT_BYTES = 9,
-       SPNG_CFG_COUNT = 10 };
+       SPNG_CFG_RESOLVE_WINDOW = 10,
+       SPNG_CFG_COUNT = 11 };
 enum { SPNG_BLOCK_CUT_AUTO = 0, SPNG_BLOCK_CUT_NEVER = 1 };
+enum { SPNG_WINDOW_AUTO = 0, SPNG_WINDOW_NARROW = 1, SPNG_WINDOW_WIDE = 2 };
 enum { SPNG_INFLATE_AUTO = 0, SPNG_INFLATE_SERIAL = 1 };
 int32_t spng_configure(spng_ctx *ctx, int key, int64_t value);
 
@@ -133,6 +135,7 @@
 int32_t spng_profile_get(spng_ctx *ctx, int kernel, double *total_ms, uint64_t *launches);
 int32_t spng_token_stats(spng_ctx *ctx, uint64_t *page_bytes, uint64_t *blocks, int32_t *ran_dry);
 int32_t spng_cut_stats(spng_ctx *ctx, uint64_t *tried, uint64_t *joined, uint64_t *streams_redone);
+int32_t spng_window_stats(spng_ctx *ctx, uint64_t *narrow, uint64_t *wide);
 
 int32_t spng_inflate_batch(spng_ctx *ctx, const spng_stream_desc *descs, uint32_t count,
                            spng_result *d_results, spng_result *h_results);
diff --git a/swift_png_amd/__init__.py b/swift_png_amd/__init__.py
--- a/swift_png_amd/__init__.py
+++ b/swift_png_amd/__init__.py
@@ -51,12 +51,14 @@
 CFG_DEFLATE_BYTES, CFG_MULTI_GROUPS = 7, 8
 CFG_BLOCK_CUT_BYTES = 9
 BLOCK_CUT_AUTO, BLOCK_CUT_NEVER = 0, 1
+CFG_RESOLVE_WINDOW = 10
+WINDOW_AUTO, WINDOW_NARROW, WINDOW_WIDE = 0, 1, 2
 INFLATE_AUTO, INFLATE_SERIAL = 0, 1
 
 EXPORTS = [
     "spng_version", "spng_status_string", "spng_last_error_string", "spng_inflated_size",
     "spng_storage_size", "spng_create", "spng_destroy", "spng_stream", "spng_sync", "spng_profile",
-    "spng_profile_get", "spng_token_stats", "spng_cut_stats", "spng_configure", "spng_inflate_batch", "spng_inflate_resume_batch", "spng_unfilter_batch",
+    "spng_profile_get", "spng_token_stats", "spng_cut_stats", "spng_window_stats", "spng_configure", "spng_inflate_batch", "spng_inflate_resume_batch", "spng_unfilter_batch",
     "spng_unfilter_resume_batch", "spng_decode_batch",
     "spng_inflate", "spng_unfilter", "spng_decode", "spng_adler32", "spng_filter_batch", "spng_filter",
     "spng_lex_batch", "spng_write_idat_batch", "spng_crc32", "spng_unpack_batch", "spng_unpack", "spng_unpack_as", "spng_pack_batch", "spng_pack_as", "spng_alpha_batch", "spng_alpha", "spng_hsva_batch", "spng_hsva", "spng_luminance_batch", "spng_luminance", "spng_census_batch", "spng_census", "spng_pack_indexed_batch", "spng_pack_indexed", "spng_census_wide_batch", "spng_census_wide", "spng_map_batch", "spng_map", "spng_deflate_bound", "spng_deflate_batch", "spng_deflate", "spng_deflate_window", "spng_encode_batch",
@@ -324,6 +326,7 @@
     lib.spng_profile_get.argtypes = [vp, ctypes.c_int, ctypes.POINTER(ctypes.c_double), ctypes.POINTER(u64)]
     lib.spng_token_stats.argtypes = [vp, ctypes.POINTER(u64), ctypes.POINTER(u64), ctypes.POINTER(ctypes.c_int32)]
     lib.spng_cut_stats.argtypes = [vp, ctypes.POINTER(u64), ctypes.POINTER(u64), ctypes.POINTER(u64)]
+    lib.spng_window_stats.argtypes = [vp, ctypes.POINTER(u64), ctypes.POINTER(u64)]
     lib.spng_inflate_batch.argtypes = [vp, ctypes.POINTER(StreamDesc), u32, vp, rp]
     lib.spng_inflate_resume_batch.argtypes = [vp, ctypes.POINTER(StreamDesc), ctypes.POINTER(ctypes.c_uint64), u32, vp, rp]
     lib.spng_unfilter_batch.argtypes = [vp, ctypes.POINTER(ImageDesc), u32, vp, vp, rp]
@@ -561,6 +564,11 @@
         _check(self.lib, self.lib.spng_cut_stats(self.ctx, ctypes.byref(t), ctypes.byref(j), ctypes.byref(r)))
         return t.value, j.value, r.value
 
+    def window_stats(self):
+        a, b = ctypes.c_uint64(0), ctypes.c_uint64(0)
+        _check(self.lib, self.lib.spng_window_stats(self.ctx, ctypes.byref(a), ctypes.byref(b)))
+        return a.value, b.value
+
     def to_device(self, data):
         t = self.torch
         if isinstance(data, (bytes, bytearray, memoryview)):
diff --git a/swift_png_amd/csrc/api.hip b/swift_png_amd/csrc/api.hip
--- a/swift_png_amd/csrc/api.hip
+++ b/swift_png_amd/csrc/api.hip
@@ -159,6 +159,7 @@
 int32_t spng_configure(spng_ctx *c, int key, int64_t value)
 {
     if (!c || key < 0 || key >= SPNG_CFG_COUNT || key == 4 || key == 6  || value < 0) return SPNG_E_ARGUMENT;
+    if (key == SPNG_CFG_RESOLVE_WINDOW && value > SPNG_WINDOW_WIDE) return SPNG_E_ARGUMENT;
     std::lock_guard<std::mutex> g(c->mu);
     c->cfg[key] = value;
     return SPNG_DONE;
@@ -198,6 +199,18 @@
     if (tried) *tried = h ? h[0] : 0;
     if (joined) *joined = h ? h[1] : 0;
     if (streams_redone) *streams_redone = h ? h[2] : 0;
+    return SPNG_DONE;
+}
+
+int32_t spng_window_stats(spng_ctx *c, uint64_t *narrow, uint64_t *wide)
+{
+    if (!c) return SPNG_E_ARGUMENT;
+    std::lock_guard<std::mutex> g(c->mu);
+    HIP_TRY(hipSetDevice(c->device));
+    HIP_TRY(hipStreamSynchronize(c->stream));
+    const uint32_t *h = c->h_pool_used ? c->h_pool_used + 12 : nullptr;
+    if (narrow) *narrow = h ? h[0] : 0;
+    if (wide) *wide = h ? h[1] : 0;
     return SPNG_DONE;
 }
 
diff --git a/swift_png_amd/csrc/common.hpp b/swift_png_amd/csrc/common.hpp
--- a/swift_png_amd/csrc/common.hpp
+++ b/swift_png_amd/csrc/common.hpp
@@ -220,7 +220,9 @@
     uint32_t       cut_on, cut_resumed;
     uint64_t       seg_origin, tok_bit, blk_out;
     uint64_t       ho_hdr, ho_out;
-};
+    uint32_t       win_cfg, wide;
+};
+static constexpr uint64_t R_WIDE_NUM = 7, R_WIDE_DEN = 5;
 enum { PSEG_FAIL = 0, PSEG_CONT = 1, PSEG_FINAL = 2, PSEG_PARTIAL = 3, PSEG_NOPAGE = 4,
        PSEG_CUT = 5 };
 static constexpr uint64_t RESUME_SERIAL_BITS = 8ull << 20;
@@ -342,11 +344,11 @@
 hipError_t launch_pinf2_find(PStream *d_streams, PSeg *d_segs, uint32_t seg0, uint32_t nsegs, uint32_t retry, hipStream_t stream);
 hipError_t launch_pinf2_decode(PStream *d_streams, PSeg *d_segs, uint32_t seg0, uint32_t nsegs, uint32_t *d_pt, uint8_t *d_pool, uint32_t *d_next,
                                uint32_t pages, uint32_t retry, hipStream_t stream);
-hipError_t launch_pinf2_scan(PStream *d_streams, uint32_t nstreams, PSeg *d_segs, PPart *d_parts, uint32_t retry, hipStream_t stream);
+hipError_t launch_pinf2_scan(PStream *d_streams, uint32_t nstreams, PSeg *d_segs, PPart *d_parts, uint32_t *d_wstats, uint32_t retry, hipStream_t stream);
 hipError_t launch_pinf2_resolve(PStream *d_streams, uint32_t nstreams, PSeg *d_segs, uint32_t *d_pt, uint8_t *d_pool, uint32_t pages,
-                                spng_result *d_results, int32_t *d_done, PPart *d_parts, uint32_t pmax, uint32_t retry, hipStream_t stream);
+                                spng_result *d_results, int32_t *d_done, PPart *d_parts, uint32_t pmax, uint32_t retry, uint32_t classes, hipStream_t stream);
 hipError_t launch_pinf2_parts(PStream *d_streams, uint32_t nstreams, PSeg *d_segs, uint32_t *d_pt, uint8_t *d_pool, uint32_t pages,
-                              spng_result *d_results, int32_t *d_done, PPart *d_parts, uint32_t pmax, uint16_t *d_sym, hipStream_t stream);
+                              spng_result *d_results, int32_t *d_done, PPart *d_parts, uint32_t pmax, uint16_t *d_sym, uint32_t classes, hipStream_t stream);
 hipError_t launch_pinf2_join(PStream *d_streams, uint32_t nstreams, spng_result *d_results, int32_t *d_done, PPart *d_parts, uint32_t pmax,
                              uint16_t *d_sym, uint8_t *d_win, hipStream_t stream);
 hipError_t launch_pinf2_cutplan(PStream *d_streams, uint32_t nstreams, PSeg *d_segs, PCut *d_cuts, uint32_t *d_stats, hipStream_t stream);
@@ -354,7 +356,8 @@
                                   uint32_t *d_next, uint32_t pages, hipStream_t stream);
 hipError_t launch_pinf2_cutjoin(PStream *d_streams, PSeg *d_segs, PCut *d_cuts, uint32_t seg0, uint32_t nsegs, uint32_t *d_pt, uint8_t *d_pool,
                                 uint32_t *d_next, uint32_t pages, uint32_t *d_stats, hipStream_t stream);
-hipError_t launch_pinf2_cutscan(PStream *d_streams, uint32_t nstreams, PSeg *d_segs, PCut *d_cuts, PPart *d_parts, uint32_t *d_stats, hipStream_t stream);
+hipError_t launch_pinf2_cutscan(PStream *d_streams, uint32_t nstreams, PSeg *d_segs, PCut *d_cuts, PPart *d_parts, uint32_t *d_stats, uint32_t *d_wstats,
+                                hipStream_t stream);
 hipError_t launch_pinf2_account(uint32_t *d_ctr, uint32_t *d_totals, uint32_t pages, hipStream_t stream);
 static constexpr uint64_t GZ_NONE = ~0ull;
 uint32_t   gzip_pieces();
diff --git a/swift_png_amd/csrc/host.hpp b/swift_png_amd/csrc/host.hpp
--- a/swift_png_amd/csrc/host.hpp
+++ b/swift_png_amd/csrc/host.hpp
@@ -71,7 +71,7 @@
     hipEvent_t ev_out[2] = {nullptr, nullptr};
     void *d_multi = nullptr; size_t multi_cap = 0;
     uint64_t peers = 0, peers_refused = 0;
-    int64_t cfg[SPNG_CFG_COUNT] = {0, 0, 0, 0, 0, 0, 0, 0, 0};
+    int64_t cfg[SPNG_CFG_COUNT] = {0, 0, 0, 0, 0, 0, 0, 0, 0, 0, 0};
     bool profiling = false;
     struct Span { int kernel; hipEvent_t a, b; };
     std::vector<Span> spans;
diff --git a/swift_png_amd/csrc/host_decode.hip b/swift_png_amd/csrc/host_decode.hip
--- a/swift_png_amd/csrc/host_decode.hip
+++ b/swift_png_amd/csrc/host_decode.hip
@@ -201,6 +201,7 @@
         memset(&st, 0, sizeof st);
         st.src = j.src; st.dst = j.dst; st.src_len = j.src_len; st.dst_cap = j.dst_cap;
         st.format = j.format; st.image = j.image;
+        st.win_cfg = (uint32_t)c->cfg[SPNG_CFG_RESOLVE_WINDOW];
         const int64_t cb = c->cfg[SPNG_CFG_BLOCK_CUT_BYTES];
         const uint64_t cut_bytes = cb == 0 ? RESUME_SERIAL_BITS / 8 : (uint64_t)cb;
         uint64_t origin = 0;
@@ -392,8 +393,8 @@
         memcpy(a.host<PSeg>(p.segs_at), p.segs.data(), p.segs.size() * sizeof(PSeg));
     }
     if (p.parallel) {
-        p.next_at = a.take(64);
-        memset(a.host<uint32_t>(p.next_at), 0, 64);
+        p.next_at = a.take(128);
+        memset(a.host<uint32_t>(p.next_at), 0, 128);
         if (p.pmax) {
             p.parts_at = a.take(n * p.pmax * sizeof(PPart));
             memset(a.host<PPart>(p.parts_at), 0, n * p.pmax * sizeof(PPart));
@@ -486,17 +487,19 @@
             { Timed t(c, SPNG_K_PINF_DECODE, q); HIP_TRY(launch_pinf2_decode(ds, dg, g.g0, g.g1 - g.g0, dlog, pool, dnext, pages, retry, q)); }
             PPart *dparts = p.pmax ? a.dev<PPart>(p.parts_at) + (size_t)g.s0 * p.pmax : nullptr;
             const uint32_t pm = retry ? 0u : p.pmax;
-            if (cuts) HIP_TRY(launch_pinf2_cutscan(ds + g.s0, g.s1 - g.s0, dg, dc, dparts, dnext + 12, q));
-            else HIP_TRY(launch_pinf2_scan(ds + g.s0, g.s1 - g.s0, dg, dparts, retry, q));
+            if (cuts) HIP_TRY(launch_pinf2_cutscan(ds + g.s0, g.s1 - g.s0, dg, dc, dparts, dnext + 12, dnext + 16, q));
+            else HIP_TRY(launch_pinf2_scan(ds + g.s0, g.s1 - g.s0, dg, dparts, dnext + 16, retry, q));
+            const int64_t wcfg = c->cfg[SPNG_CFG_RESOLVE_WINDOW];
+            const uint32_t classes = wcfg == SPNG_WINDOW_NARROW ? 1u : wcfg == SPNG_WINDOW_WIDE ? 2u : 3u;
             {
                 Timed t(c, SPNG_K_PINF_RESOLVE, q);
                 if (pm) {
                     if (int32_t st = second_stream(c)) return st;
                     HIP_TRY(hipEventRecord(c->ev_fork, q));
                     HIP_TRY(hipStreamWaitEvent(c->stream2, c->ev_fork, 0));
-                    HIP_TRY(launch_pinf2_parts(ds + g.s0, g.s1 - g.s0, dg, dlog, pool, pages, dr, dd + g.s0, dparts, pm, (uint16_t *)c->d_sym, c->stream2));
+                    HIP_TRY(launch_pinf2_parts(ds + g.s0, g.s1 - g.s0, dg, dlog, pool, pages, dr, dd + g.s0, dparts, pm, (uint16_t *)c->d_sym, classes, c->stream2));
                 }
-                HIP_TRY(launch_pinf2_resolve(ds + g.s0, g.s1 - g.s0, dg, dlog, pool, pages, dr, dd + g.s0, dparts, pm, retry, q));
+                HIP_TRY(launch_pinf2_resolve(ds + g.s0, g.s1 - g.s0, dg, dlog, pool, pages, dr, dd + g.s0, dparts, pm, retry, classes, q));
                 if (pm) {
                     HIP_TRY(hipEventRecord(c->ev_join, c->stream2));
                     HIP_TRY(hipStreamWaitEvent(q, c->ev_join, 0));
@@ -506,7 +509,7 @@
             }
             HIP_TRY(launch_pinf2_account(dnext, dnext + 8, pages, q));
         }
-        if (c->cut_stats_valid) HIP_TRY(hipMemcpyAsync(c->h_pool_used + 8, dnext + 12, 12, hipMemcpyDeviceToHost, c->stream));
+        HIP_TRY(hipMemcpyAsync(c->h_pool_used + 8, dnext + 12, 24, hipMemcpyDeviceToHost, c->stream));
         if (!c->pool_pending) {
             HIP_TRY(hipMemcpyAsync(c->h_pool_used, dnext + 8, 16, hipMemcpyDeviceToHost, c->stream));
             c->pool_src_pending = c->pool_src_bytes;
diff --git a/swift_png_amd/csrc/pinflate2.hip b/swift_png_amd/csrc/pinflate2.hip
--- a/swift_png_amd/csrc/pinflate2.hip
+++ b/swift_png_amd/csrc/pinflate2.hip
@@ -25,6 +25,7 @@
 typedef uint8_t AS_GLOBAL g8;
 typedef uint16_t AS_GLOBAL g16;
 typedef uint32_t AS_GLOBAL g32;
+typedef uint64_t AS_GLOBAL g64;
 typedef PV4 AS_GLOBAL gPV4;
 typedef uint32_t v2u __attribute__((vector_size(8)));
 struct __attribute__((packed)) PV2 { v2u v; };
@@ -68,7 +69,7 @@
 #endif
 
 #if defined(SPNG_EMU) && defined(SPNG_EMU_COV)
-static long g_cov[13];
+static long g_cov[14];
 #define COV(k) __atomic_fetch_add(&g_cov[k], 1, __ATOMIC_RELAXED)
 #else
 #define COV(k) ((void)0)
@@ -1233,7 +1234,7 @@
 
 template <uint32_t RETRY, bool CUT>
 __device__ __forceinline__ void scan_stream(PStream *__restrict__ streams, PSeg *__restrict__ segs, PPart *__restrict__ parts, uint32_t *__restrict__ stats,
-                                            const PCut *__restrict__ cuts)
+                                            const PCut *__restrict__ cuts, uint32_t *__restrict__ wstats)
 {
     constexpr uint32_t retry = RETRY;
     const int lane = threadIdx.x;
@@ -1340,19 +1341,23 @@
         }
         if (lane == 0) { pp[np - 1].seg_end = ~0u; pp[np - 1].out_len = out - begun; }
     }
+    const uint32_t wcfg = UNI(st.win_cfg);
+    const bool wide = wcfg == SPNG_WINDOW_WIDE || (wcfg != SPNG_WINDOW_NARROW && tok * 2 * R_WIDE_DEN > out * R_WIDE_NUM);
     if (lane == 0) { st.ok = ok ? (handed ? 3 : partial ? 2 : 1) : 0; st.ntok = tok; st.end_bit = end_bit; st.pass = again ? 1 : 0; st.tok_base = 0;
-                     st.out_total = out; st.parts = np; st.ho_hdr = cur_hdr; st.ho_out = cur_out; }
+                     st.out_total = out; st.parts = np; st.ho_hdr = cur_hdr; st.ho_out = cur_out; st.wide = wide ? 1 : 0;
+                     if (ok && !retry && wstats) atomicAdd(wstats + (wide ? 1 : 0), 1u); }
 }
 
 template <uint32_t RETRY>
-__global__ __launch_bounds__(64) void pinf2_scan_kernel(PStream *__restrict__ streams, PSeg *__restrict__ segs, PPart *__restrict__ parts)
-{
-    scan_stream<RETRY, false>(streams, segs, parts, nullptr, nullptr);
+__global__ __launch_bounds__(64) void pinf2_scan_kernel(PStream *__restrict__ streams, PSeg *__restrict__ segs, PPart *__restrict__ parts,
+                                                        uint32_t *__restrict__ wstats = nullptr)
+{
+    scan_stream<RETRY, false>(streams, segs, parts, nullptr, nullptr, wstats);
 }
 __global__ __launch_bounds__(64) void pinf2_cutscan_kernel(PStream *__restrict__ streams, PSeg *__restrict__ segs, const PCut *__restrict__ cuts,
-                                                           PPart *__restrict__ parts, uint32_t *__restrict__ stats)
-{
-    scan_stream<0, true>(streams, segs, parts, stats, cuts);
+                                                           PPart *__restrict__ parts, uint32_t *__restrict__ stats, uint32_t *__restrict__ wstats = nullptr)
+{
+    scan_stream<0, true>(streams, segs, parts, stats, cuts, wstats);
 }
 
 #ifndef SPNG_R_THREADS
@@ -1361,16 +1366,20 @@
 #endif
 static constexpr uint32_t RT2 = SPNG_R_THREADS;
 static constexpr uint32_t NW2 = RT2 / 64;
-template <bool BIG> struct RGeo {
+template <bool BIG, bool WIDE = false> struct RGeo {
     static constexpr uint32_t TILE = BIG ? 8192 : 4096;
     static constexpr uint32_t BPT = TILE / RT2;
-    static constexpr uint32_t HPT = TILE / 2 / RT2;
+    static constexpr uint32_t HPT = TILE / 2 / RT2 * (WIDE ? 2 : 1);
+    static constexpr uint32_t UH = HPT < 8 ? HPT : 8;
     static constexpr uint32_t EB = BPT < 8 ? BPT : 8;
     static constexpr uint32_t MAXM = TILE / 8;
 };
 static constexpr uint32_t WINDOW2 = 32768;
 static constexpr uint32_t R2_DONE = 0x8000;
-static constexpr uint32_t PTC = 256;
+#ifndef SPNG_R_PTC
+#define SPNG_R_PTC 256
+#endif
+static constexpr uint32_t PTC = SPNG_R_PTC;
 
 template <bool MARK> struct RingOf { typedef uint8_t T; };
 template <> struct RingOf<true> { typedef uint16_t T; };
@@ -1410,7 +1419,7 @@
 {
     const g8 *src = (const g8 *)st.src;
     const uint64_t n = st.src_len;
-    uint64_t *state = st.state;
+    g64 *state = (g64 *)st.state;
     const bool whole = st.start_bit == 0 && st.out_pos == 0;
     if (st.ok == 2 || st.ok == 3) {
         const bool tok = st.ok == 3;
@@ -1445,15 +1454,17 @@
     }
 }
 
-template <uint32_t RETRY, bool MARK, bool BIG>
-__global__ __launch_bounds__(RT2, SPNG_R_WAVES) void pinf2_resolve_kernel(const PStream *__restrict__ streams, const PSeg *__restrict__ segs,
-                                                               const uint32_t *__restrict__ pt_slab, DPool pool,
-                                                               spng_result *__restrict__ results, int32_t *__restrict__ done,
-                                                               PPart *__restrict__ parts, uint32_t pmax, uint16_t *__restrict__ sym)
+template <uint32_t RETRY, bool MARK, bool BIG, bool WIDE>
+__device__ __forceinline__ void resolve_stream(const PStream *__restrict__ streams, const PSeg *__restrict__ segs,
+                                               const uint32_t *__restrict__ pt_slab, DPool pool,
+                                               spng_result *__restrict__ results, int32_t *__restrict__ done,
+                                               PPart *__restrict__ parts, uint32_t pmax, uint16_t *__restrict__ sym)
 {
     constexpr uint32_t retry = RETRY;
-    constexpr uint32_t TILE2 = RGeo<BIG>::TILE, BPT2 = RGeo<BIG>::BPT, HPT2 = RGeo<BIG>::HPT, EB2 = RGeo<BIG>::EB, MAXM2 = RGeo<BIG>::MAXM;
-    static_assert(HPT2 == 8 || HPT2 == 4, "a thread's halfwords of a window are one 16- or 8-byte load");
+    typedef RGeo<BIG, WIDE> Geo;
+    constexpr uint32_t TILE2 = Geo::TILE, BPT2 = Geo::BPT, HPT2 = Geo::HPT, UH2 = Geo::UH, EB2 = Geo::EB, MAXM2 = Geo::MAXM;
+    static_assert(UH2 == 8 || (UH2 == 4 && HPT2 == 4), "a thread's halfwords of a window are 16-byte loads, or one 8-byte load");
+    static_assert((1u << 20) / 258 > MAXM2 + 1 && RT2 * HPT2 / 2 <= 1u << 12, "the packed scan of the take");
     constexpr uint32_t DONE = MARK ? 0x4000u : R2_DONE;
     constexpr uint32_t KNOWN = MARK ? 0xc000u : R2_DONE;
     __shared__ __attribute__((aligned(16))) RLds2T<MARK, BIG> s;
@@ -1462,6 +1473,7 @@
     const uint32_t pidx = MARK ? 1 + blockIdx.x % (pmax - 1) : 0;
     const PStream &st = streams[sidx];
     if (!UNI(st.ok) || (retry && done[sidx])) return;
+    if ((UNI(st.wide) != 0) != WIDE) return;
     const uint32_t nparts = pmax ? UNI(st.parts) : 0;
     if (MARK && pidx >= nparts) return;
     PPart *part = nparts > 1 ? parts + (uint64_t)sidx * pmax + pidx : nullptr;
@@ -1503,34 +1515,49 @@
         __syncthreads();
         uint32_t tv[HPT2 / 2];
         auto load_window = [&](uint64_t from) {
-            const uint64_t h = (from & ~(uint64_t)(HPT2 - 1)) + (uint64_t)tid * HPT2;
+            const uint64_t hfirst = (from & ~(uint64_t)(UH2 - 1)) + (uint64_t)tid * HPT2;
 #pragma unroll
             for (int k = 0; k < (int)(HPT2 / 2); ++k) tv[k] = NULL2;
-            if (h < nhw) {
-                const uint64_t u = h >> 3;
-                const uint32_t pid = s.pt[(u >> (PAGE_SHIFT - 4)) - pt_lo];
-                const g8 *q = (const g8 *)pool.base + ((uint64_t)pid << PAGE_SHIFT) + ((u & (PAGE_UNITS - 1)) << 4) + ((h & 7) << 1);
-                if constexpr (HPT2 == 8) { const v4u v = ((const gPV4 *)q)->v; tv[0] = v[0]; tv[1] = v[1]; tv[2] = v[2]; tv[3] = v[3]; }
-                else { const v2u v = ((const gPV2 *)q)->v; tv[0] = v[0]; tv[1] = v[1]; }
+#pragma unroll
+            for (int n = 0; n < (int)(HPT2 / UH2); ++n) {
+                const uint64_t h = hfirst + (uint64_t)n * UH2;
+                if (h < nhw) {
+                    const uint64_t u = h >> 3;
+                    const uint32_t pid = s.pt[(u >> (PAGE_SHIFT - 4)) - pt_lo];
+                    const g8 *q = (const g8 *)pool.base + ((uint64_t)pid << PAGE_SHIFT) + ((u & (PAGE_UNITS - 1)) << 4) + ((h & 7) << 1);
+                    if constexpr (UH2 == 8) { const v4u v = ((const gPV4 *)q)->v; tv[4 * n] = v[0]; tv[4 * n + 1] = v[1]; tv[4 * n + 2] = v[2]; tv[4 * n + 3] = v[3]; }
+                    else { const v2u v = ((const gPV2 *)q)->v; tv[0] = v[0]; tv[1] = v[1]; }
+                }
             }
         };
         load_window(cursor);
         while (cursor < nhw) {
             RP2(0);
             const uint64_t wb = cursor;
-            uint32_t hh[HPT2];
+            uint32_t hh[WIDE ? 1 : HPT2];
+            if constexpr (WIDE) {
+                const uint64_t mine = wb + (uint32_t)tid * HPT2;
+                const uint32_t nv = mine >= nhw ? 0u : nhw - mine < HPT2 ? (uint32_t)(nhw - mine) : HPT2;
+#pragma unroll
+                for (int k = 0; k < (int)(HPT2 / 2); ++k) tv[k] = 2 * k + 1 < (int)nv ? tv[k] : 2 * k < (int)nv ? tv[k] | TK_NULL << 16 : NULL2;
+            } else {
 #pragma unroll
             for (int j = 0; j < (int)HPT2; ++j) {
                 const uint32_t idx = (uint32_t)tid * HPT2 + j;
                 const uint32_t v = (tv[j >> 1] >> (16 * (j & 1))) & 0xffff;
                 hh[j] = wb + idx < nhw ? v : TK_NULL;
             }
-            s.h0[tid] = (uint16_t)hh[0];
+            }
+            auto hw = [&](int j) -> uint32_t {
+                if constexpr (WIDE) return (tv[j >> 1] >> (16 * (j & 1))) & 0xffff;
+                else return hh[j];
+            };
+            s.h0[tid] = (uint16_t)hw(0);
             if (tid == 0) s.cut[1] = 0xffffffffu;
             uint32_t bytes = 0, refs = 0;
 #pragma unroll
             for (int j = 0; j < (int)HPT2; ++j) {
-                const uint32_t v = hh[j];
+                const uint32_t v = hw(j);
                 const bool lit = !(v & 0x8000), m0 = (v & 0xC000) == 0x8000;
                 bytes += lit ? 1u : m0 ? (v & 0xff) + 3 : 0u;
                 refs += m0 ? 1u : 0u;
@@ -1542,16 +1569,16 @@
             const uint32_t hnext = tid + 1 < (int)RT2 ? s.h0[tid + 1] : TK_NULL;
             const bool front = curb <= TILE2 && curm <= MAXM2;
             const bool fits = curb + bytes <= TILE2 && curm + refs <= MAXM2 &&
-                              !(tid == (int)RT2 - 1 && (hh[HPT2 - 1] & 0xC000) == 0x8000);
+                              !(tid == (int)RT2 - 1 && (hw(HPT2 - 1) & 0xC000) == 0x8000);
             if (front && !fits) { s.cut[0] = curb; s.cut[1] = (uint32_t)tid * HPT2; if (curb + bytes <= TILE2 && curm + refs > MAXM2) COV(9); }
             if (fits) {
 #pragma unroll
                 for (int j = 0; j < (int)HPT2; ++j) {
-                    const uint32_t v = hh[j];
+                    const uint32_t v = hw(j);
                     if (!(v & 0x8000)) { s.state[curb] = (uint16_t)(DONE | v); curb += 1; }
                     else if ((v & 0xC000) == 0x8000) {
                         const uint32_t len = (v & 0xff) + 3;
-                        const uint32_t h1 = j < (int)HPT2 - 1 ? hh[j < (int)HPT2 - 1 ? j + 1 : (int)HPT2 - 1] : hnext;
+                        const uint32_t h1 = j < (int)HPT2 - 1 ? hw(j < (int)HPT2 - 1 ? j + 1 : (int)HPT2 - 1) : hnext;
                         const uint32_t dd = (((v >> 8) & 63) | (h1 & 0x1ff) << 6) + 1;
                         atomicOr(&s.bitmap[curb >> 5], 1u << (curb & 31));
                         s.rec[curm + 1][0] = curb | len << 16;
@@ -1569,6 +1596,7 @@
             const uint64_t cursor_next = wb + wlast;
             if ((((cursor_next + 2 * RT2 * HPT2) >> 3) >> (PAGE_SHIFT - 4)) >= pt_lo + PTC) {
                 __syncthreads();
+                COV(13);
                 pt_lo = (cursor_next >> 3) >> (PAGE_SHIFT - 4);
                 for (uint32_t i = (uint32_t)tid; i < PTC; i += RT2) s.pt[i] = (pt_lo + i) * PAGE_UNITS * 8 < nhw + 8 ? ptg[pt_lo + i] : 0u;
                 __syncthreads();
@@ -1744,6 +1772,22 @@
         if (tid == 0) stream_verdict(st, S, I, pos, results, done + sidx);
     }
 }
+template <uint32_t RETRY, bool MARK, bool BIG>
+__global__ __launch_bounds__(RT2, SPNG_R_WAVES) void pinf2_resolve_kernel(const PStream *__restrict__ streams, const PSeg *__restrict__ segs,
+                                                               const uint32_t *__restrict__ pt_slab, DPool pool,
+                                                               spng_result *__restrict__ results, int32_t *__restrict__ done,
+                                                               PPart *__restrict__ parts, uint32_t pmax, uint16_t *__restrict__ sym)
+{
+    resolve_stream<RETRY, MARK, BIG, false>(streams, segs, pt_slab, pool, results, done, parts, pmax, sym);
+}
+template <uint32_t RETRY, bool MARK, bool BIG>
+__global__ __launch_bounds__(RT2, SPNG_R_WAVES) void pinf2_resolve_wide_kernel(const PStream *__restrict__ streams, const PSeg *__restrict__ segs,
+                                                               const uint32_t *__restrict__ pt_slab, DPool pool,
+                                                               spng_result *__restrict__ results, int32_t *__restrict__ done,
+                                                               PPart *__restrict__ parts, uint32_t pmax, uint16_t *__restrict__ sym)
+{
+    resolve_stream<RETRY, MARK, BIG, true>(streams, segs, pt_slab, pool, results, done, parts, pmax, sym);
+}
 
 __global__ __launch_bounds__(512) void pinf2_window_kernel(const PStream *__restrict__ streams, const PPart *__restrict__ parts, uint32_t pmax,
                                                            const uint16_t *__restrict__ sym, uint8_t *__restrict__ win)
@@ -1884,31 +1928,45 @@
     pinf2_cutjoin_kernel<<<nsegs, 64, 0, stream>>>(d_streams, d_segs, d_cuts, d_pt, pool, seg0, d_stats);
     return hipGetLastError();
 }
-hipError_t launch_pinf2_cutscan(PStream *d_streams, uint32_t nstreams, PSeg *d_segs, PCut *d_cuts, PPart *d_parts, uint32_t *d_stats, hipStream_t stream)
-{
-    pinf2_cutscan_kernel<<<nstreams, 64, 0, stream>>>(d_streams, d_segs, d_cuts, d_parts, d_stats);
+hipError_t launch_pinf2_cutscan(PStream *d_streams, uint32_t nstreams, PSeg *d_segs, PCut *d_cuts, PPart *d_parts, uint32_t *d_stats, uint32_t *d_wstats,
+                                hipStream_t stream)
+{
+    pinf2_cutscan_kernel<<<nstreams, 64, 0, stream>>>(d_streams, d_segs, d_cuts, d_parts, d_stats, d_wstats);
     return hipGetLastError();
 }
-hipError_t launch_pinf2_scan(PStream *d_streams, uint32_t nstreams, PSeg *d_segs, PPart *d_parts, uint32_t retry, hipStream_t stream)
-{
-    if (retry) pinf2_scan_kernel<1><<<nstreams, 64, 0, stream>>>(d_streams, d_segs, d_parts);
-    else pinf2_scan_kernel<0><<<nstreams, 64, 0, stream>>>(d_streams, d_segs, d_parts);
+hipError_t launch_pinf2_scan(PStream *d_streams, uint32_t nstreams, PSeg *d_segs, PPart *d_parts, uint32_t *d_wstats, uint32_t retry, hipStream_t stream)
+{
+    if (retry) pinf2_scan_kernel<1><<<nstreams, 64, 0, stream>>>(d_streams, d_segs, d_parts, d_wstats);
+    else pinf2_scan_kernel<0><<<nstreams, 64, 0, stream>>>(d_streams, d_segs, d_parts, d_wstats);
     return hipGetLastError();
 }
 hipError_t launch_pinf2_resolve(PStream *d_streams, uint32_t nstreams, PSeg *d_segs, uint32_t *d_pt, uint8_t *d_pool, uint32_t pages,
-                                spng_result *d_results, int32_t *d_done, PPart *d_parts, uint32_t pmax, uint32_t retry, hipStream_t stream)
+                                spng_result *d_results, int32_t *d_done, PPart *d_parts, uint32_t pmax, uint32_t retry, uint32_t classes, hipStream_t stream)
 {
     DPool pool{d_pool, nullptr, pages, 0};
-    if (retry) pinf2_resolve_kernel<1, false, true><<<nstreams, RT2, 0, stream>>>(d_streams, d_segs, d_pt, pool, d_results, d_done, d_parts, pmax, nullptr);
-    else pinf2_resolve_kernel<0, false, true><<<nstreams, RT2, 0, stream>>>(d_streams, d_segs, d_pt, pool, d_results, d_done, d_parts, pmax, nullptr);
+    if (classes & 1) {
+        if (retry) pinf2_resolve_kernel<1, false, true><<<nstreams, RT2, 0, stream>>>(d_streams, d_segs, d_pt, pool, d_results, d_done, d_parts, pmax, nullptr);
+        else pinf2_resolve_kernel<0, false, true><<<nstreams, RT2, 0, stream>>>(d_streams, d_segs, d_pt, pool, d_results, d_done, d_parts, pmax, nullptr);
+    }
+    if (classes & 2) {
+        if (retry) pinf2_resolve_wide_kernel<1, false, true><<<nstreams, RT2, 0, stream>>>(d_streams, d_segs, d_pt, pool, d_results, d_done, d_parts, pmax, nullptr);
+        else pinf2_resolve_wide_kernel<0, false, true><<<nstreams, RT2, 0, stream>>>(d_streams, d_segs, d_pt, pool, d_results, d_done, d_parts, pmax, nullptr);
+    }
     return hipGetLastError();
 }
 hipError_t launch_pinf2_parts(PStream *d_streams, uint32_t nstreams, PSeg *d_segs, uint32_t *d_pt, uint8_t *d_pool, uint32_t pages,
-                              spng_result *d_results, int32_t *d_done, PPart *d_parts, uint32_t pmax, uint16_t *d_sym, hipStream_t stream)
+                              spng_result *d_results, int32_t *d_done, PPart *d_parts, uint32_t pmax, uint16_t *d_sym, uint32_t classes, hipStream_t stream)
 {
     DPool pool{d_pool, nullptr, pages, 0};
-    if (nstreams * (pmax - 1) > 256) pinf2_resolve_kernel<0, true, false><<<nstreams * (pmax - 1), RT2, 0, stream>>>(d_streams, d_segs, d_pt, pool, d_results, d_done, d_parts, pmax, d_sym);
-    else pinf2_resolve_kernel<0, true, true><<<nstreams * (pmax - 1), RT2, 0, stream>>>(d_streams, d_segs, d_pt, pool, d_results, d_done, d_parts, pmax, d_sym);
+    const bool small = nstreams * (pmax - 1) > 256;
+    if (classes & 1) {
+        if (small) pinf2_resolve_kernel<0, true, false><<<nstreams * (pmax - 1), RT2, 0, stream>>>(d_streams, d_segs, d_pt, pool, d_results, d_done, d_parts, pmax, d_sym);
+        else pinf2_resolve_kernel<0, true, true><<<nstreams * (pmax - 1), RT2, 0, stream>>>(d_streams, d_segs, d_pt, pool, d_results, d_done, d_parts, pmax, d_sym);
+    }
+    if (classes & 2) {
+        if (small) pinf2_resolve_wide_kernel<0, true, false><<<nstreams * (pmax - 1), RT2, 0, stream>>>(d_streams, d_segs, d_pt, pool, d_results, d_done, d_parts, pmax, d_sym);
+        else pinf2_resolve_wide_kernel<0, true, true><<<nstreams * (pmax - 1), RT2, 0, stream>>>(d_streams, d_segs, d_pt, pool, d_results, d_done, d_parts, pmax, d_sym);
+    }
     return hipGetLastError();
 }
 hipError_t launch_pinf2_join(PStream *d_streams, uint32_t nstreams, spng_result *d_results, int32_t *d_done, PPart *d_parts, uint32_t pmax,
```

Measured after the change: 35750. About the same (-0.2%).
